# aclyde11/molecular-VAE

Measured on AMD Instinct MI355X. Metric: molecules/s (ELBO fwd+bwd+step), higher is better.
Workload: dtype bf16

## Files before the change

### molecular-vae_amd/csrc/capi.hip

```cpp
#include "common.hpp"
#include "kernels.hpp"

int rnn_fwd_impl(const mvae_rnn_fwd_desc* d, hipStream_t st);
int rnn_bwd_impl(const mvae_rnn_bwd_desc* d, hipStream_t st);
size_t rnn_bwd_workspace_bytes(const mvae_rnn_bwd_desc* d);

thread_local const void* mvae_tls_status = nullptr;

extern "C" {

int mvae_abi_version(void) { return MVAE_ABI_VERSION; }
size_t mvae_struct_size(int which) {
  switch (which) {
    case 0: return sizeof(mvae_rnn_fwd_desc);
    case 1: return sizeof(mvae_rnn_bwd_desc);
    case 2: return sizeof(mvae_gemm_tn_problem);
    case 3: return sizeof(mvae_pack_job);
    case 4: return sizeof(mvae_gemm_tn_f32_problem);
    default: return 0;
  }
}

int mvae_knob_int(const char* name, int dflt) {
  const char* v = name ? mvae_knob(name) : nullptr;
  return v ? atoi(v) : dflt;
}

const char* mvae_status_string(int status) {
  switch (status) {
    case MVAE_OK: return "ok";
    case MVAE_ERR_INVALID: return "invalid argument";
    case MVAE_ERR_WORKSPACE: return "workspace too small";
    case MVAE_ERR_UNSUPPORTED: return "unsupported combination";
    default: return status > 0 ? hipGetErrorString((hipError_t)status) : "unknown status";
  }
}

size_t mvae_gemm_nt_workspace(int M, int N, int K, int dtype_ab) { return gemm_nt_workspace_bytes(M, N, K, dtype_ab); }

int mvae_gemm_nt(int dtype_ab, int M, int N, int K, const void* A, int64_t lda, const void* B, int64_t ldb, void* C, int64_t ldc,
                 int dtype_c, const float* bias, int act, int accumulate, void* ws, size_t ws_bytes, void* stream) {
  return launch_gemm_nt(dtype_ab, M, N, K, A, lda, B, ldb, C, ldc, dtype_c, bias, act, accumulate, ws, ws_bytes, (hipStream_t)stream);
}

size_t mvae_gemm_tn_workspace(int M, int N, int K, int dtype_ab) {
  return dtype_ab == MVAE_BF16 ? gemm_tn_workspace_bytes(M, N, K) : dtype_ab == MVAE_F32 ? gemm_tn_f32_workspace_bytes(M, N, K) : 0;
}

int mvae_gemm_tn(int dtype_ab, int M, int N, int K, const void* A, int64_t lda, const void* B, int64_t ldb, void* C, int64_t ldc,
                 int dtype_c, const float* bias, int act, int accumulate, void* ws, size_t ws_bytes, void* stream) {
  if (dtype_ab == MVAE_F32) {
    if (dtype_c != MVAE_F32 || bias || act != MVAE_ACT_NONE) return MVAE_ERR_UNSUPPORTED;
    return launch_gemm_tn_f32(M, N, K, (const float*)A, lda, 0, 0, (const float*)B, ldb, 0, 0, (float*)C, ldc, accumulate, ws, ws_bytes, (hipStream_t)stream);
  }
  if (dtype_ab != MVAE_BF16) return MVAE_ERR_UNSUPPORTED;
  return launch_gemm_tn_bf16(M, N, K, A, lda, B, ldb, C, ldc, dtype_c, bias, act, accumulate, ws, ws_bytes, (hipStream_t)stream);
}

int mvae_gemm_tn_f32_colsum(int M, int N, int K, const float* A, int64_t lda, const float* B, int64_t ldb, float* C, int64_t ldc, int accumulate,
                            float* colsum_out, int colsum_accumulate, void* ws, size_t ws_bytes, void* stream) {
  if (!colsum_out) return MVAE_ERR_INVALID;
  return launch_gemm_tn_f32(M, N, K, A, lda, 0, 0, B, ldb, 0, 0, C, ldc, accumulate, ws, ws_bytes, (hipStream_t)stream, false, colsum_out, colsum_accumulate);
}

size_t mvae_gemm_tn_colsum_workspace(int M, int N, int K) { return gemm_tn_colsum_supported(M, N, K) ? gemm_tn_colsum_workspace_bytes(M, N, K) : 0; }
int mvae_gemm_tn_colsum_supported(int M, int N, int K) { return gemm_tn_colsum_supported(M, N, K) ? 1 : 0; }
int mvae_gemm_tn_colsum(int M, int N, int K, const void* A, int64_t lda, const void* B, int64_t ldb, float* C, int64_t ldc, int accumulate,
                        float* colsum_out, int colsum_accumulate, void* ws, size_t ws_bytes, void* stream) {
  if (!colsum_out) return MVAE_ERR_INVALID;
  return launch_gemm_tn_bf16_colsum(M, N, K, A, lda, B, ldb, C, ldc, MVAE_F32, nullptr, MVAE_ACT_NONE, accumulate, colsum_out, colsum_accumulate,
                                    ws, ws_bytes, (hipStream_t)stream);
}

int mvae_dropout_keep(uint32_t seed, uint32_t idx, float p) {
  uint32_t h = idx * 0x9E3779B1u ^ seed;
  h ^= h >> 16; h *= 0x85EBCA6Bu; h ^= h >> 13; h *= 0xC2B2AE35u; h ^= h >> 16;
  return h >= (uint32_t)((double)p * 4294967296.0) ? 1 : 0;
}

int mvae_rnn_fwd(const mvae_rnn_fwd_desc* d, void* stream, const void** status_out) {
  mvae_tls_status = nullptr;
  const int rc = (d && d->persist_ws && !d->no_spin && rnn_persist_fwd_supported(d))
                     ? rnn_persist_fwd(d, d->persist_ws, d->persist_ws_bytes, (hipStream_t)stream)
                     : rnn_fwd_impl(d, (hipStream_t)stream);
  if (status_out) *status_out = rc == MVAE_OK ? mvae_tls_status : nullptr;
  return rc;
}
size_t mvae_rnn_fwd_persist_workspace(const mvae_rnn_fwd_desc* d) {
  if (!d) return 0;
  if (rnn_persist_fwd_supported(d)) return rnn_persist_fwd_workspace_bytes(d->T);
  return rnn_rowres_fwd_pipe_workspace(d);
}
int mvae_rnn_bwd(const mvae_rnn_bwd_desc* d, void* stream, const void** status_out) {
  mvae_tls_status = nullptr;
  const int rc = (d && d->persist_ws && !d->no_spin && rnn_persist_bwd_supported(d))
                     ? rnn_persist_bwd(d, d->persist_ws, d->persist_ws_bytes, (hipStream_t)stream)
                     : rnn_bwd_impl(d, (hipStream_t)stream);
  if (status_out) *status_out = rc == MVAE_OK ? mvae_tls_status : nullptr;
  return rc;
}
size_t mvae_rnn_bwd_persist_workspace(const mvae_rnn_bwd_desc* d) { return (d && rnn_persist_bwd_supported(d)) ? rnn_persist_bwd_workspace_bytes(d->T) : 0; }
size_t mvae_rnn_bwd_workspace(const mvae_rnn_bwd_desc* d) { return rnn_bwd_workspace_bytes(d); }

}
```

### molecular-vae_amd/csrc/kernels.hpp

```cpp
#pragma once
#include <atomic>
#include <hip/hip_runtime.h>
#include <stddef.h>
#include "../../include/mvae.h"

size_t gemm_nt_workspace_bytes(int M, int N, int K, int dtype);
int launch_gemm_nt(int dtype, int M, int N, int K, const void* A, long lda, const void* B, long ldb, void* C, long ldc,
                   int c_dtype, const float* bias, int act, int accumulate, void* ws, size_t ws_bytes, hipStream_t st);
int launch_gemm_nt_grouped(int dtype, int M, int N, int K, const void* A, long lda, int a_group, long a_gstride, long a_total,
                           const void* B, long ldb, void* C, long ldc, int c_dtype, const float* bias, int act, int accumulate,
                           void* ws, size_t ws_bytes, hipStream_t st);
size_t gemm_tn_f32_workspace_bytes(int M, int N, int R);
int launch_gemm_tn_f32(int M, int N, int R, const float* A, long lda, int a_group, long a_gstride, const float* B, long ldb, int b_group,
                       long b_gstride, float* C, long ldc, int accumulate, void* ws, size_t ws_bytes, hipStream_t st, bool x3 = false,
                       float* colsum_out = nullptr, int colsum_acc = 0);
size_t gemm_tn_workspace_bytes(int M, int N, int K);
int launch_gemm_tn_bf16(int M, int N, int K, const void* A, long lda, const void* B, long ldb, void* C, long ldc, int c_dtype,
                        const float* bias, int act, int accumulate, void* ws, size_t ws_bytes, hipStream_t st);
bool gemm_tn_colsum_supported(int M, int N, int K);
size_t gemm_tn_colsum_workspace_bytes(int M, int N, int K);
int launch_gemm_tn_bf16_colsum(int M, int N, int K, const void* A, long lda, const void* B, long ldb, void* C, long ldc, int c_dtype,
                               const float* bias, int act, int accumulate, float* colsum_out, int colsum_acc, void* ws, size_t ws_bytes,
                               hipStream_t st);
int launch_cast_transpose(int dsrc, int ddst, int R, int C, const void* src, long lds_, void* dst, long ldd, void* dstT,
                          long ldt, hipStream_t st);
size_t colsum_workspace_bytes(int M, int N);
int launch_colsum(int M, int N, const float* X, long ldx, float* out, void* ws, size_t ws_bytes, hipStream_t st);
int launch_selu_bwd(long n, float* dy, const float* y, hipStream_t st);

extern thread_local const void* mvae_tls_status;
constexpr int MVAE_MAX_DEVICES = 64;

bool rnn_persist_fwd_supported(const mvae_rnn_fwd_desc* d);
size_t rnn_persist_fwd_workspace_bytes(int T);
int rnn_persist_fwd(const mvae_rnn_fwd_desc* d, void* ws, size_t ws_bytes, hipStream_t st);
bool rnn_persist_bwd_supported(const mvae_rnn_bwd_desc* d);
size_t rnn_persist_bwd_workspace_bytes(int T);
int rnn_persist_bwd(const mvae_rnn_bwd_desc* d, void* ws, size_t ws_bytes, hipStream_t st);
size_t rnn_rowres_fwd_pipe_workspace(const mvae_rnn_fwd_desc* d);
```

### molecular-vae_amd/csrc/rnn.hip

```cpp
#include "tile_pipe.hpp"
#include "kernels.hpp"
#include <stdlib.h>

template <typename T> __device__ __forceinline__ void load8(const T* p, float (&v)[8]);
template <> __device__ __forceinline__ void load8<float>(const float* p, float (&v)[8]) {
  const float4 a = *reinterpret_cast<const float4*>(p), b = *reinterpret_cast<const float4*>(p + 4);
  v[0] = a.x; v[1] = a.y; v[2] = a.z; v[3] = a.w; v[4] = b.x; v[5] = b.y; v[6] = b.z; v[7] = b.w;
}
template <> __device__ __forceinline__ void load8<bf16_t>(const bf16_t* p, float (&v)[8]) {
  const uint4 u = *reinterpret_cast<const uint4*>(p);
  const uint32_t w[4] = {u.x, u.y, u.z, u.w};
#pragma unroll
  for (int i = 0; i < 4; ++i) { v[2 * i] = __builtin_bit_cast(float, w[i] << 16); v[2 * i + 1] = __builtin_bit_cast(float, w[i] & 0xffff0000u); }
}
template <typename T> __device__ __forceinline__ void store8(T* p, const float (&v)[8]);
template <> __device__ __forceinline__ void store8<float>(float* p, const float (&v)[8]) {
  *reinterpret_cast<float4*>(p) = make_float4(v[0], v[1], v[2], v[3]);
  *reinterpret_cast<float4*>(p + 4) = make_float4(v[4], v[5], v[6], v[7]);
}
template <> __device__ __forceinline__ void store8<bf16_t>(bf16_t* p, const float (&v)[8]) {
  uint4 u;
  u.x = (uint32_t)f2bf(v[0]) | ((uint32_t)f2bf(v[1]) << 16); u.y = (uint32_t)f2bf(v[2]) | ((uint32_t)f2bf(v[3]) << 16);
  u.z = (uint32_t)f2bf(v[4]) | ((uint32_t)f2bf(v[5]) << 16); u.w = (uint32_t)f2bf(v[6]) | ((uint32_t)f2bf(v[7]) << 16);
  *reinterpret_cast<uint4*>(p) = u;
}
template <typename T> __device__ __forceinline__ void ldn(const T* p, float (&v)[8], int n, bool vec) {
  if (vec && n == 8) { load8<T>(p, v); return; }
#pragma unroll
  for (int e = 0; e < 8; ++e) v[e] = (e < n) ? TT<T>::ld(p + e) : 0.f;
}
template <typename T> __device__ __forceinline__ void stn(T* p, const float (&v)[8], int n, bool vec) {
  if (vec && n == 8) { store8<T>(p, v); return; }
#pragma unroll
  for (int e = 0; e < 8; ++e) if (e < n) TT<T>::st(p + e, v[e]);
}

template <typename T> __device__ __forceinline__ float act_sigmoid(float x);
template <typename T> __device__ __forceinline__ float act_tanh(float x);
template <> __device__ __forceinline__ float act_sigmoid<float>(float x) { return 1.f / (1.f + expf(-x)); }
template <> __device__ __forceinline__ float act_tanh<float>(float x) { return tanhf(x); }
template <> __device__ __forceinline__ float act_sigmoid<bf16_t>(float x) { return __builtin_amdgcn_rcpf(1.f + __expf(-x)); }
template <> __device__ __forceinline__ float act_tanh<bf16_t>(float x) { return fmaf(-2.f, __builtin_amdgcn_rcpf(1.f + __expf(2.f * x)), 1.f); }

__device__ __forceinline__ int xcd_remap_r(int bid, int n) {
  const int q = n >> 3, r = n & 7, x = bid & 7, i = bid >> 3;
  return (x < r ? x * (q + 1) : r * (q + 1) + (x - r) * q) + i;
}

struct DropArgs { float scale; uint32_t thresh, seed; };
__host__ __device__ __forceinline__ uint32_t drop_hash(uint32_t seed, uint32_t idx) {
  uint32_t h = idx * 0x9E3779B1u ^ seed;
  h ^= h >> 16; h *= 0x85EBCA6Bu; h ^= h >> 13; h *= 0xC2B2AE35u; h ^= h >> 16;
  return h;
}
__device__ __forceinline__ float drop_factor(const DropArgs& da, const uint8_t* mask, uint32_t idx0, long off) {
  const bool keep = mask ? (mask[off] != 0) : (drop_hash(da.seed, idx0 + (uint32_t)off) >= da.thresh);
  return keep ? da.scale : 0.f;
}

struct StepTaskF {
  const void *A0, *A1, *W0, *W1;
  long lda0, lda1, ldw0, ldw1;
  int K0, K1;
  const float* add; long add_ld;
  const float* add_tbl;
  const int64_t* add_idx; long add_idx_ld; int add_rows;
  const float* bias;
  const float* c_prev; float* c_out;
  void* c_save;
  void* h_out; long ldh;
  void* g_out;
  const void* hprev_t0;
  int t;
  void* h_drop;
  const uint8_t* dmask;
  uint32_t didx0;
};
struct StepArgsF { StepTaskF t[MVAE_MAX_LAYERS]; const int* lengths; int ntask, B, H, tiles_m, tiles_j, dbg, vec, cell, gru3; DropArgs drop; };

template <typename T, int BM, int BJ, int NBUF, bool WS = false>
__global__ __launch_bounds__(WS ? 512 : 256) void lstm_step_fwd_kernel(StepArgsF p) {
  constexpr bool PIPE = NBUF > 0;
  constexpr int NTHR = WS ? 512 : 256;
  static_assert(!WS || NBUF > 0, "wave specialisation needs the LDS-direct ring");
  extern __shared__ __attribute__((aligned(16))) char smem[];
  static_assert(BJ == 32 || BJ == 64, "hidden units per tile");
  constexpr int JS = BJ / 32;
  constexpr int BN = 4 * BJ, WM = BM / 2, MI = WM / 16, NI = 4 * JS;
  const int tid = threadIdx.x, lane = tid & 63, wave = (tid >> 6) & 3, wm = wave >> 1, wj = wave & 1;
  const int per_task = p.tiles_m * p.tiles_j;
  const int bid = xcd_remap_r(blockIdx.x, p.ntask * per_task);
  const int task = bid / per_task;
  const int rem = bid - task * per_task;
  const int tj = rem / p.tiles_m, tm = rem - tj * p.tiles_m;
  const StepTaskF& q = p.t[task];
  const int m0 = tm * BM, j0 = tj * BJ, H = p.H, B = p.B;

  f32x4 acc[MI][NI];
#pragma unroll
  for (int i = 0; i < MI; ++i)
#pragma unroll
    for (int g = 0; g < NI; ++g) acc[i][g] = f32x4{0.f, 0.f, 0.f, 0.f};

#ifdef MVAE_TUNING
  const bool run_main = !(p.dbg & 2);
#else
  constexpr bool run_main = true;
#endif
  if (run_main) {
  if constexpr (PIPE) {
    PipeSeg<BM, BN> s0, s1;
    const uint32_t sz = (uint32_t)sizeof(T);
    const int skip0 = p.gru3 ? 3 : -1, skip1 = p.gru3 ? 2 : -1;
    {
      const uint32_t lda = (uint32_t)q.lda0 * sz, ldw = (uint32_t)q.ldw0 * sz;
      auto offA = [&](int r) -> uint32_t { const int gm = m0 + r; return gm < B ? (uint32_t)gm * lda : PIPE_OOB; };
      auto offB = [&](int r) -> uint32_t { const int g = r / BJ, j = j0 + (r - g * BJ); return (j < H && g != skip0) ? (uint32_t)(g * H + j) * ldw : PIPE_OOB; };
      pipe_seg_init<T, BM, BN>(s0, q.A0, (uint32_t)B * lda, q.W0, (uint32_t)(4 * H) * ldw, offA, offB, q.K0, tid & 255);
    }
    {
      const uint32_t lda = (uint32_t)q.lda1 * sz, ldw = (uint32_t)q.ldw1 * sz;
      auto offA = [&](int r) -> uint32_t { const int gm = m0 + r; return gm < B ? (uint32_t)gm * lda : PIPE_OOB; };
      auto offB = [&](int r) -> uint32_t { const int g = r / BJ, j = j0 + (r - g * BJ); return (j < H && g != skip1) ? (uint32_t)(g * H + j) * ldw : PIPE_OOB; };
      pipe_seg_init<T, BM, BN>(s1, q.A1, (uint32_t)B * lda, q.W1, (uint32_t)(4 * H) * ldw, offA, offB, q.K1, tid & 255);
    }
    if constexpr (WS) tile_gemm_ws<T, BM, BN, MI, NI, (NBUF > 0 ? NBUF : 3), JS, BJ>(smem, s0, s1, wm * WM, wj * (BJ / 2), acc, tid);
    else tile_gemm_pipe<T, BM, BN, MI, NI, (NBUF > 0 ? NBUF : 3), JS, BJ>(smem, s0, s1, wm * WM, wj * (BJ / 2), acc, tid);
  } else {
    int brow[NI];
#pragma unroll
    for (int g = 0; g < NI; ++g) brow[g] = (g / JS) * BJ + wj * (BJ / 2) + (g % JS) * 16;
    if (q.A0 != nullptr) {
      const T* A = reinterpret_cast<const T*>(q.A0);
      const T* W = reinterpret_cast<const T*>(q.W0);
      const long lda = q.lda0, ldw = q.ldw0;
      auto rowA = [&](int r) -> const T* { const int gm = m0 + r; return gm < B ? A + (long)gm * lda : nullptr; };
      auto rowB = [&](int r) -> const T* { const int g = r / BJ, j = j0 + (r - g * BJ); return (j < H && !(p.gru3 && g == 3)) ? W + ((long)g * H + j) * ldw : nullptr; };
      tile_gemm_segment<T, BM, BN, MI, NI>(smem, rowA, rowB, 0, q.K0, wm * WM, brow, acc, tid);
    }
    if (q.A1 != nullptr) {
      const T* A = reinterpret_cast<const T*>(q.A1);
      const T* W = reinterpret_cast<const T*>(q.W1);
      const long lda = q.lda1, ldw = q.ldw1;
      auto rowA = [&](int r) -> const T* { const int gm = m0 + r; return gm < B ? A + (long)gm * lda : nullptr; };
      auto rowB = [&](int r) -> const T* { const int g = r / BJ, j = j0 + (r - g * BJ); return (j < H && !(p.gru3 && g == 2)) ? W + ((long)g * H + j) * ldw : nullptr; };
      tile_gemm_segment<T, BM, BN, MI, NI>(smem, rowA, rowB, 0, q.K1, wm * WM, brow, acc, tid);
    }
  }
  }
#ifdef MVAE_TUNING
  if (p.dbg & 1) { if (acc[0][0][0] == 12345.678f) q.c_out[0] = 1.f; return; }
#endif

  constexpr int SJ = BJ + 4;
  constexpr int GPRW = BJ / 8;
  constexpr int NIT = (BM * GPRW + NTHR - 1) / NTHR;
  float* stg = reinterpret_cast<float*>(smem);
  const int g8 = tid % GPRW;
  const int j8 = j0 + g8 * 8;
  const int n = (H - j8 < 8) ? (H - j8) : 8;
  const bool vec = p.vec != 0;
  const bool fast = vec && n == 8 && m0 + BM <= B && (BM * GPRW) % NTHR == 0;
  float bias[4][8], cpv[NIT][8];
  if (fast) {
    const float* bsrc = q.bias ? q.bias : q.c_out;
#pragma unroll
    for (int g = 0; g < 4; ++g) load8<float>(bsrc + g * H + j8, bias[g]);
    if (q.c_prev) {
#pragma unroll
      for (int it = 0; it < NIT; ++it) load8<float>(q.c_prev + (long)(m0 + tid / GPRW + it * (NTHR / GPRW)) * H + j8, cpv[it]);
    } else if (q.hprev_t0) {
#pragma unroll
      for (int it = 0; it < NIT; ++it)
        load8<T>(reinterpret_cast<const T*>(q.hprev_t0) + (long)(m0 + tid / GPRW + it * (NTHR / GPRW)) * q.lda1 + j8, cpv[it]);
    } else {
#pragma unroll
      for (int it = 0; it < NIT; ++it)
#pragma unroll
        for (int e = 0; e < 8; ++e) cpv[it][e] = 0.f;
    }
    if (!q.bias) {
#pragma unroll
      for (int g = 0; g < 4; ++g)
#pragma unroll
        for (int e = 0; e < 8; ++e) bias[g][e] = 0.f;
    }
  } else {
#pragma unroll
  for (int g = 0; g < 4; ++g) {
    if (q.bias && n > 0) ldn<float>(q.bias + g * H + j8, bias[g], n, vec);
    else {
#pragma unroll
      for (int e = 0; e < 8; ++e) bias[g][e] = 0.f;
    }
  }
#pragma unroll
  for (int it = 0; it < NIT; ++it) {
    const int lrow = tid / GPRW + it * (NTHR / GPRW);
    const int row = m0 + lrow;
    const bool live = n > 0 && lrow < BM && row < B;
    if (live && q.c_prev) ldn<float>(q.c_prev + (long)row * H + j8, cpv[it], n, vec);
    else if (live && q.hprev_t0) ldn<T>(reinterpret_cast<const T*>(q.hprev_t0) + (long)row * q.lda1 + j8, cpv[it], n, vec);
    else {
#pragma unroll
      for (int e = 0; e < 8; ++e) cpv[it][e] = 0.f;
    }
  }
  }
  if (!WS || tid < 256) {
    const int lr = lane & 15, lq = lane >> 4;
#pragma unroll
    for (int i = 0; i < MI; ++i)
#pragma unroll
      for (int ni = 0; ni < NI; ++ni)
#pragma unroll
        for (int r = 0; r < 4; ++r) {
          const int row = wm * WM + i * 16 + lq * 4 + r;
          stg[(row * 4 + ni / JS) * SJ + wj * (BJ / 2) + (ni % JS) * 16 + lr] = acc[i][ni][r];
        }
  }
  __syncthreads();
  if (n <= 0) return;
  T* hout = reinterpret_cast<T*>(q.h_out);
  T* gout = reinterpret_cast<T*>(q.g_out);
  T* csave = reinterpret_cast<T*>(q.c_save);
  auto rows = [&](auto fast_tag, auto add_tag) {
  constexpr bool FAST = decltype(fast_tag)::value, HAS_ADD = decltype(add_tag)::value;
  auto ld32 = [&](const float* src, float (&v)[8]) { if constexpr (FAST) load8<float>(src, v); else ldn<float>(src, v, n, vec); };
  auto st32 = [&](float* dst, const float (&v)[8]) { if constexpr (FAST) store8<float>(dst, v); else stn<float>(dst, v, n, vec); };
  auto stT = [&](T* dst, const float (&v)[8]) { if constexpr (FAST) store8<T>(dst, v); else stn<T>(dst, v, n, vec); };
#pragma unroll
  for (int it = 0; it < NIT; ++it) {
    const int lrow = tid / GPRW + it * (NTHR / GPRW);
    const int row = m0 + lrow;
    if constexpr (!FAST) { if (lrow >= BM || row >= B) continue; }
    float pre[4][8];
#pragma unroll
    for (int g = 0; g < 4; ++g) {
      const float* s = stg + (lrow * 4 + g) * SJ + g8 * 8;
      const float4 a = *reinterpret_cast<const float4*>(s), b = *reinterpret_cast<const float4*>(s + 4);
      pre[g][0] = a.x + bias[g][0]; pre[g][1] = a.y + bias[g][1]; pre[g][2] = a.z + bias[g][2]; pre[g][3] = a.w + bias[g][3];
      pre[g][4] = b.x + bias[g][4]; pre[g][5] = b.y + bias[g][5]; pre[g][6] = b.z + bias[g][6]; pre[g][7] = b.w + bias[g][7];
    }
    if constexpr (HAS_ADD) {
    if (q.add_tbl) {
      long id = q.add_idx[(long)row * q.add_idx_ld];
      id = id < 0 ? 0 : (id >= q.add_rows ? q.add_rows - 1 : id);
      const float* tr = q.add_tbl + id * 4L * H + j8;
#pragma unroll
      for (int g = 0; g < 4; ++g) {
        float a[8], b[8];
        ld32(tr + g * H, a);
        if (q.add) {
          ld32(q.add + (long)row * q.add_ld + g * H + j8, b);
#pragma unroll
          for (int e = 0; e < 8; ++e) a[e] += b[e];
        }
#pragma unroll
        for (int e = 0; e < 8; ++e) pre[g][e] += a[e];
      }
    } else if (q.add) {
#pragma unroll
      for (int g = 0; g < 4; ++g) {
        float a[8];
        ld32(q.add + (long)row * q.add_ld + g * H + j8, a);
#pragma unroll
        for (int e = 0; e < 8; ++e) pre[g][e] += a[e];
      }
    }
    }
    const float (&cp)[8] = cpv[it];
    T* g4 = gout + (long)row * 4 * H + j8;
    if (p.cell == MVAE_CELL_LSTM) {
      float gi[8], gf[8], gg[8], go[8], c[8], h[8];
#pragma unroll
      for (int e = 0; e < 8; ++e) {
        gi[e] = act_sigmoid<T>(pre[0][e]); gf[e] = act_sigmoid<T>(pre[1][e]); gg[e] = act_tanh<T>(pre[2][e]); go[e] = act_sigmoid<T>(pre[3][e]);
        c[e] = gf[e] * cp[e] + gi[e] * gg[e];
        h[e] = go[e] * act_tanh<T>(c[e]);
      }
      st32(q.c_out + (long)row * H + j8, c);
      stT(hout + (long)row * q.ldh + j8, h);
      if (q.h_drop) {
        float hd[8];
#pragma unroll
        for (int e = 0; e < 8; ++e) hd[e] = (e < n) ? h[e] * drop_factor(p.drop, q.dmask, q.didx0, (long)row * H + j8 + e) : 0.f;
        stT(reinterpret_cast<T*>(q.h_drop) + (long)row * q.ldh + j8, hd);
      }
      if (gout) {
        stT(csave + (long)row * H + j8, c);
        stT(g4, gi); stT(g4 + H, gf); stT(g4 + 2 * H, gg); stT(g4 + 3 * H, go);
      }
    } else {
      const bool valid = p.lengths ? (q.t < p.lengths[row]) : true;
      float gr[8], gz[8], gn[8], hs_[8], hseq[8];
#pragma unroll
      for (int e = 0; e < 8; ++e) {
        gr[e] = act_sigmoid<T>(pre[0][e]); gz[e] = act_sigmoid<T>(pre[1][e]);
        gn[e] = act_tanh<T>(pre[2][e] + gr[e] * pre[3][e]);
        const float hn = (1.f - gz[e]) * gn[e] + gz[e] * cp[e];
        hs_[e] = valid ? hn : cp[e];
        hseq[e] = valid ? hn : 0.f;
      }
      st32(q.c_out + (long)row * H + j8, hs_);
      stT(hout + (long)row * q.ldh + j8, hseq);
      if (q.h_drop) {
        float hd[8];
#pragma unroll
        for (int e = 0; e < 8; ++e) hd[e] = (e < n) ? hseq[e] * drop_factor(p.drop, q.dmask, q.didx0, (long)row * H + j8 + e) : 0.f;
        stT(reinterpret_cast<T*>(q.h_drop) + (long)row * q.ldh + j8, hd);
      }
      if (gout) { stT(g4, gr); stT(g4 + H, gz); stT(g4 + 2 * H, gn); stT(g4 + 3 * H, pre[3]); }
    }
  }
  };
  const bool has_add = q.add != nullptr || q.add_tbl != nullptr;
  if (fast) { if (has_add) rows(std::true_type{}, std::true_type{}); else rows(std::true_type{}, std::false_type{}); }
  else { if (has_add) rows(std::false_type{}, std::true_type{}); else rows(std::false_type{}, std::false_type{}); }
}

template <int BMW, int BNB, int NBUF, bool WS = false>
__global__ __launch_bounds__(WS ? 512 : BMW * 2) void lstm_step_fwd_gm_kernel(StepArgsF p) {
  using T = bf16_t;
  extern __shared__ __attribute__((aligned(16))) char smem[];
  static_assert(BMW == 256 || BMW == 128, "weight rows per tile: 64 or 32 units x 4 gates");
  static_assert(!WS || BMW == 128, "loader / consumer split: the 4-wave tile only");
  constexpr int NT = BMW * 2;
  constexpr int BU = BMW / 4;
  constexpr int MI = 8, NI = BNB / 64;
  const int tid = threadIdx.x, lane = tid & 63, wave = WS ? ((tid >> 6) & 3) : (tid >> 6), wm = wave >> 2, wn = wave & 3;
  const int per_task = p.tiles_m * p.tiles_j;
  const int bid = xcd_remap_r(blockIdx.x, p.ntask * per_task);
  const int task = bid / per_task;
  const int rem = bid - task * per_task;
  const int tj = rem / p.tiles_m, tm = rem - tj * p.tiles_m;
  const StepTaskF& q = p.t[task];
  const int n0 = tm * BNB, j0 = tj * BU, H = p.H, B = p.B;

  const int lq = lane >> 4, lc = lane & 15;
  const int ub = j0 + 32 * wm + 8 * lq;
  constexpr bool BIAS_FIRST = (BMW == 256 && BNB == 256);
  auto load_bias = [&](float (&bias)[4][8]) {
    if (q.bias) {
#pragma unroll
      for (int g = 0; g < 4; ++g) load8<float>(q.bias + g * H + ub, bias[g]);
    } else {
#pragma unroll
      for (int g = 0; g < 4; ++g)
#pragma unroll
        for (int e = 0; e < 8; ++e) bias[g][e] = 0.f;
    }
  };
  f32x4 acc[MI][NI];
  if constexpr (BIAS_FIRST) {
    float bias[4][8];
    load_bias(bias);
#pragma unroll
    for (int ni = 0; ni < NI; ++ni)
#pragma unroll
      for (int g = 0; g < 4; ++g)
#pragma unroll
        for (int e = 0; e < 8; ++e) acc[2 * g + (e >> 2)][ni][e & 3] = bias[g][e];
  } else {
#pragma unroll
    for (int i = 0; i < MI; ++i)
#pragma unroll
      for (int g = 0; g < NI; ++g) acc[i][g] = f32x4{0.f, 0.f, 0.f, 0.f};
  }

  float cpa[NI][8];
  auto load_cprev_all = [&]() {
    const float* cpsrc = q.c_prev ? q.c_prev : q.c_out;
#pragma unroll
    for (int ni = 0; ni < NI; ++ni) {
      const int row = n0 + wn * (16 * NI) + ni * 16 + lc;
      load8<float>(cpsrc + (long)(row < B ? row : B - 1) * H + ub, cpa[ni]);
    }
  };
  if constexpr (BIAS_FIRST) load_cprev_all();

#ifdef MVAE_TUNING
  const bool run_main = !(p.dbg & 2);
#else
  constexpr bool run_main = true;
#endif
  if (run_main) {
    PipeSeg<BMW, BNB, NT> s0, s1;
    auto wrow = [&](int r) -> int {
      const int mi = (r >> 4) & 7, j = r & 15;
      return (mi >> 1) * H + j0 + 32 * (r >> 7) + 8 * (j >> 2) + 4 * (mi & 1) + (j & 3);
    };
    {
      const uint32_t lda = (uint32_t)q.lda0 * 2u, ldw = (uint32_t)q.ldw0 * 2u;
      auto offW = [&](int r) -> uint32_t { return (uint32_t)wrow(r) * ldw; };
      auto offX = [&](int r) -> uint32_t { const int gn = n0 + r; return gn < B ? (uint32_t)gn * lda : PIPE_OOB; };
      pipe_seg_init<T, BMW, BNB, NT>(s0, q.W0, (uint32_t)(4 * H) * ldw, q.A0, (uint32_t)B * lda, offW, offX, q.K0, WS ? (tid & 255) : tid);
      if (q.A0 == nullptr) s0.nk = 0;
    }
    {
      const uint32_t lda = (uint32_t)q.lda1 * 2u, ldw = (uint32_t)q.ldw1 * 2u;
      auto offW = [&](int r) -> uint32_t { return (uint32_t)wrow(r) * ldw; };
      auto offX = [&](int r) -> uint32_t { const int gn = n0 + r; return gn < B ? (uint32_t)gn * lda : PIPE_OOB; };
      pipe_seg_init<T, BMW, BNB, NT>(s1, q.W1, (uint32_t)(4 * H) * ldw, q.A1, (uint32_t)B * lda, offW, offX, q.K1, WS ? (tid & 255) : tid);
      if (q.A1 == nullptr) s1.nk = 0;
    }
    if constexpr (WS) tile_gemm_ws<T, BMW, BNB, MI, NI, NBUF, NI, 0>(smem, s0, s1, 0, wn * (16 * NI), acc, tid);
    else tile_gemm_pipe_all<T, BMW, BNB, MI, NI, NBUF, NT>(smem, s0, s1, wm * 128, wn * (16 * NI), acc, tid);
  }
  if constexpr (WS) { if (tid >= 256) return; }
#ifdef MVAE_TUNING
  if (p.dbg & 1) { if (acc[0][0][0] == 12345.678f) q.c_out[0] = 1.f; return; }
#endif

  if constexpr (!BIAS_FIRST) {
    float bias[4][8];
    load_bias(bias);
#pragma unroll
    for (int ni = 0; ni < NI; ++ni)
#pragma unroll
      for (int g = 0; g < 4; ++g)
#pragma unroll
        for (int e = 0; e < 8; ++e) acc[2 * g + (e >> 2)][ni][e & 3] += bias[g][e];
  }
  T* hout = reinterpret_cast<T*>(q.h_out);
  T* gout = reinterpret_cast<T*>(q.g_out);
  T* csave = reinterpret_cast<T*>(q.c_save);
  if constexpr (!BIAS_FIRST) load_cprev_all();
  const bool has_cprev = q.c_prev != nullptr;
  auto epilogue = [&](auto has_add, auto full_tile) {
#pragma unroll
  for (int ni = 0; ni < NI; ++ni) {
    const int row = n0 + wn * (16 * NI) + ni * 16 + lc;
    if constexpr (!decltype(full_tile)::value) { if (row >= B) continue; }
    float cp[8];
#pragma unroll
    for (int e = 0; e < 8; ++e) cp[e] = has_cprev ? cpa[ni][e] : 0.f;
    float pre[4][8];
#pragma unroll
    for (int g = 0; g < 4; ++g)
#pragma unroll
      for (int e = 0; e < 8; ++e) pre[g][e] = acc[2 * g + (e >> 2)][ni][e & 3];
    if constexpr (decltype(has_add)::value) {
#pragma unroll
      for (int g = 0; g < 4; ++g) {
        float a[8];
        load8<float>(q.add + (long)row * q.add_ld + g * H + ub, a);
#pragma unroll
        for (int e = 0; e < 8; ++e) pre[g][e] += a[e];
      }
    }
    float gi[8], gf[8], gg[8], go[8], c[8], h[8];
#pragma unroll
    for (int e = 0; e < 8; ++e) {
      gi[e] = act_sigmoid<T>(pre[0][e]); gf[e] = act_sigmoid<T>(pre[1][e]); gg[e] = act_tanh<T>(pre[2][e]); go[e] = act_sigmoid<T>(pre[3][e]);
      c[e] = gf[e] * cp[e] + gi[e] * gg[e];
      h[e] = go[e] * act_tanh<T>(c[e]);
    }
#ifdef MVAE_TUNING
    const int srow = (p.dbg & 4) ? n0 + (row & 15) : row;
    const bool sgate = !(p.dbg & 8);
#else
    const int srow = row;
    constexpr bool sgate = true;
#endif
    store8<float>(q.c_out + (long)srow * H + ub, c);
    store8<T>(hout + (long)srow * q.ldh + ub, h);
    if (gout) {
      T* g4 = gout + (long)srow * 4 * H + ub;
      store8<T>(csave + (long)srow * H + ub, c);
      if (sgate) { store8<T>(g4, gi); store8<T>(g4 + H, gf); store8<T>(g4 + 2 * H, gg); store8<T>(g4 + 3 * H, go); }
    }
  }
  };
  const bool full = n0 + BNB <= B;
  if (q.add) { if (full) epilogue(std::true_type{}, std::true_type{}); else epilogue(std::true_type{}, std::false_type{}); }
  else { if (full) epilogue(std::false_type{}, std::true_type{}); else epilogue(std::false_type{}, std::false_type{}); }
}

struct StepTaskB {
  const void *A0, *A1, *W0, *W1;
  long lda0, lda1, ldw0, ldw1;
  int K0, K1;
  const float* dy; long dy_ld;
  const void* gates; const void* c; const void* c_prev;
  const float* dc_in; float* dc_out;
  void* dG; long ldg;
  const void* h_prev; long ldhp;
  float* dh0;
  int t;
  int seg1_full;
  int drop;
  const uint8_t* dmask;
  uint32_t didx0;
};
struct StepArgsB { StepTaskB t[MVAE_MAX_LAYERS]; const int* lengths; float* partial; int ntask, B, H, tiles_m, tiles_n, dbg, vec, cell, split, gru3; DropArgs drop; };

template <typename T>
__device__ __forceinline__ void bwd_cell_group(const StepArgsB& p, const StepTaskB& q, int row, int j8, int n, bool vec, float (&dh)[8]) {
  const int H = p.H;
  const T* gates = reinterpret_cast<const T*>(q.gates);
  const T* cs = reinterpret_cast<const T*>(q.c);
  const T* csp = reinterpret_cast<const T*>(q.c_prev);
  T* dG = reinterpret_cast<T*>(q.dG);
  const long o = (long)row * H + j8;
  float dci[8];
  if (q.dc_in) ldn<float>(q.dc_in + o, dci, n, vec);
  else {
#pragma unroll
    for (int e = 0; e < 8; ++e) dci[e] = 0.f;
  }
  if (p.cell == MVAE_CELL_LSTM) {
    if (q.dy) {
      float a[8];
      ldn<float>(q.dy + (long)row * q.dy_ld + j8, a, n, vec);
#pragma unroll
      for (int e = 0; e < 8; ++e) dh[e] += a[e];
    }
    float gi[8], gf[8], gg[8], go[8], c[8], cp[8];
    const T* g4 = gates + (long)row * 4 * H + j8;
    ldn<T>(g4, gi, n, vec); ldn<T>(g4 + H, gf, n, vec); ldn<T>(g4 + 2 * H, gg, n, vec); ldn<T>(g4 + 3 * H, go, n, vec);
    ldn<T>(cs + o, c, n, vec);
    if (csp) ldn<T>(csp + o, cp, n, vec);
    else {
#pragma unroll
      for (int e = 0; e < 8; ++e) cp[e] = 0.f;
    }
    float di[8], df[8], dg[8], dO[8], dco[8];
#pragma unroll
    for (int e = 0; e < 8; ++e) {
      const float tc = act_tanh<T>(c[e]);
      const float d_o = dh[e] * tc;
      const float dc = dh[e] * go[e] * (1.f - tc * tc) + dci[e];
      dco[e] = dc * gf[e];
      di[e] = dc * gg[e] * gi[e] * (1.f - gi[e]);
      df[e] = dc * cp[e] * gf[e] * (1.f - gf[e]);
      dg[e] = dc * gi[e] * (1.f - gg[e] * gg[e]);
      dO[e] = d_o * go[e] * (1.f - go[e]);
    }
    stn<float>(q.dc_out + o, dco, n, vec);
    T* d4 = dG + (long)row * q.ldg + j8;
    stn<T>(d4, di, n, vec); stn<T>(d4 + H, df, n, vec); stn<T>(d4 + 2 * H, dg, n, vec); stn<T>(d4 + 3 * H, dO, n, vec);
  } else {
#pragma unroll
    for (int e = 0; e < 8; ++e) dh[e] += dci[e];
    if (q.gates == nullptr) {
      stn<float>(q.dh0 + o, dh, n, vec);
      return;
    }
    const bool valid = p.lengths ? (q.t < p.lengths[row]) : true;
    float dpr[8], dpz[8], dpn[8], dpnr[8], carry[8];
    if (valid) {
      if (q.dy) {
        float a[8];
        ldn<float>(q.dy + (long)row * q.dy_ld + j8, a, n, vec);
#pragma unroll
        for (int e = 0; e < 8; ++e) dh[e] += a[e];
      }
      float gr[8], gz[8], gn[8], nh[8], hp[8];
      const T* g4 = gates + (long)row * 4 * H + j8;
      ldn<T>(g4, gr, n, vec); ldn<T>(g4 + H, gz, n, vec); ldn<T>(g4 + 2 * H, gn, n, vec); ldn<T>(g4 + 3 * H, nh, n, vec);
      if (q.h_prev) ldn<T>(reinterpret_cast<const T*>(q.h_prev) + (long)row * q.ldhp + j8, hp, n, vec);
      else {
#pragma unroll
        for (int e = 0; e < 8; ++e) hp[e] = 0.f;
      }
#pragma unroll
      for (int e = 0; e < 8; ++e) {
        const float dn = dh[e] * (1.f - gz[e]);
        const float dz = dh[e] * (hp[e] - gn[e]);
        dpn[e] = dn * (1.f - gn[e] * gn[e]);
        dpr[e] = dpn[e] * nh[e] * gr[e] * (1.f - gr[e]);
        dpz[e] = dz * gz[e] * (1.f - gz[e]);
        dpnr[e] = dpn[e] * gr[e];
        carry[e] = dh[e] * gz[e];
      }
    } else {
#pragma unroll
      for (int e = 0; e < 8; ++e) { dpr[e] = 0.f; dpz[e] = 0.f; dpn[e] = 0.f; dpnr[e] = 0.f; carry[e] = dh[e]; }
    }
    stn<float>(q.dc_out + o, carry, n, vec);
    T* d4 = dG + (long)row * q.ldg + j8;
    stn<T>(d4, dpr, n, vec); stn<T>(d4 + H, dpz, n, vec); stn<T>(d4 + 2 * H, dpn, n, vec); stn<T>(d4 + 3 * H, dpnr, n, vec);
  }
}

struct BwdOps { float dci[8], dy[8], g[4][8], c[8], cp[8]; };

template <typename T, bool FAST>
__device__ __forceinline__ void bwd_cell_load(const StepArgsB& p, const StepTaskB& q, int row, int j8, int n, bool vec, BwdOps& r) {
  const int H = p.H;
  const T* gates = reinterpret_cast<const T*>(q.gates);
  const long o = (long)row * H + j8;
  if constexpr (FAST) {
    load8<float>((q.dc_in ? q.dc_in : q.dc_out) + o, r.dci);
    if (gates == nullptr) return;
    load8<float>(q.dy ? q.dy + (long)row * q.dy_ld + j8 : q.dc_out + o, r.dy);
    const T* g4 = gates + (long)row * 4 * H + j8;
    load8<T>(g4, r.g[0]); load8<T>(g4 + H, r.g[1]); load8<T>(g4 + 2 * H, r.g[2]); load8<T>(g4 + 3 * H, r.g[3]);
    if (p.cell == MVAE_CELL_LSTM) {
      const T* cs = reinterpret_cast<const T*>(q.c);
      const T* csp = reinterpret_cast<const T*>(q.c_prev);
      load8<T>(cs + o, r.c);
      load8<T>((csp ? csp : cs) + o, r.cp);
    } else {
      load8<T>(q.h_prev ? reinterpret_cast<const T*>(q.h_prev) + (long)row * q.ldhp + j8 : g4, r.cp);
    }
  } else {
    if (q.dc_in) ldn<float>(q.dc_in + o, r.dci, n, vec);
    if (gates == nullptr) return;
    if (q.dy) ldn<float>(q.dy + (long)row * q.dy_ld + j8, r.dy, n, vec);
    const T* g4 = gates + (long)row * 4 * H + j8;
    ldn<T>(g4, r.g[0], n, vec); ldn<T>(g4 + H, r.g[1], n, vec); ldn<T>(g4 + 2 * H, r.g[2], n, vec); ldn<T>(g4 + 3 * H, r.g[3], n, vec);
    if (p.cell == MVAE_CELL_LSTM) {
      ldn<T>(reinterpret_cast<const T*>(q.c) + o, r.c, n, vec);
      if (q.c_prev) ldn<T>(reinterpret_cast<const T*>(q.c_prev) + o, r.cp, n, vec);
    } else if (q.h_prev) ldn<T>(reinterpret_cast<const T*>(q.h_prev) + (long)row * q.ldhp + j8, r.cp, n, vec);
  }
}

template <typename T, bool FAST>
__device__ __forceinline__ void bwd_cell_finish(const StepArgsB& p, const StepTaskB& q, int row, int j8, int n, bool vec, const BwdOps& r,
                                                float (&dh)[8]) {
  const int H = p.H;
  T* dG = reinterpret_cast<T*>(q.dG);
  const long o = (long)row * H + j8;
  auto st32 = [&](float* dst, const float (&v)[8]) { if constexpr (FAST) store8<float>(dst, v); else stn<float>(dst, v, n, vec); };
  auto stT = [&](T* dst, const float (&v)[8]) { if constexpr (FAST) store8<T>(dst, v); else stn<T>(dst, v, n, vec); };
  const bool has_dci = q.dc_in != nullptr, has_dy = q.dy != nullptr;
  float dci[8];
#pragma unroll
  for (int e = 0; e < 8; ++e) dci[e] = has_dci ? r.dci[e] : 0.f;
  if (p.cell == MVAE_CELL_LSTM) {
#pragma unroll
    for (int e = 0; e < 8; ++e) dh[e] += has_dy ? r.dy[e] : 0.f;
    const bool has_cp = q.c_prev != nullptr;
    float di[8], df[8], dg[8], dO[8], dco[8];
#pragma unroll
    for (int e = 0; e < 8; ++e) {
      const float gi = r.g[0][e], gf = r.g[1][e], gg = r.g[2][e], go = r.g[3][e], cp = has_cp ? r.cp[e] : 0.f;
      const float tc = act_tanh<T>(r.c[e]);
      const float d_o = dh[e] * tc;
      const float dc = dh[e] * go * (1.f - tc * tc) + dci[e];
      dco[e] = dc * gf;
      di[e] = dc * gg * gi * (1.f - gi);
      df[e] = dc * cp * gf * (1.f - gf);
      dg[e] = dc * gi * (1.f - gg * gg);
      dO[e] = d_o * go * (1.f - go);
    }
    st32(q.dc_out + o, dco);
    T* d4 = dG + (long)row * q.ldg + j8;
    stT(d4, di); stT(d4 + H, df); stT(d4 + 2 * H, dg); stT(d4 + 3 * H, dO);
  } else {
#pragma unroll
    for (int e = 0; e < 8; ++e) dh[e] += dci[e];
    if (q.gates == nullptr) {
      st32(q.dh0 + o, dh);
      return;
    }
    const bool valid = p.lengths ? (q.t < p.lengths[row]) : true;
    const bool has_hp = q.h_prev != nullptr;
    float dpr[8], dpz[8], dpn[8], dpnr[8], carry[8];
    if (valid) {
#pragma unroll
      for (int e = 0; e < 8; ++e) dh[e] += has_dy ? r.dy[e] : 0.f;
#pragma unroll
      for (int e = 0; e < 8; ++e) {
        const float gr = r.g[0][e], gz = r.g[1][e], gn = r.g[2][e], nh = r.g[3][e], hp = has_hp ? r.cp[e] : 0.f;
        const float dn = dh[e] * (1.f - gz);
        const float dz = dh[e] * (hp - gn);
        dpn[e] = dn * (1.f - gn * gn);
        dpr[e] = dpn[e] * nh * gr * (1.f - gr);
        dpz[e] = dz * gz * (1.f - gz);
        dpnr[e] = dpn[e] * gr;
        carry[e] = dh[e] * gz;
      }
    } else {
#pragma unroll
      for (int e = 0; e < 8; ++e) { dpr[e] = 0.f; dpz[e] = 0.f; dpn[e] = 0.f; dpnr[e] = 0.f; carry[e] = dh[e]; }
    }
    st32(q.dc_out + o, carry);
    T* d4 = dG + (long)row * q.ldg + j8;
    stT(d4, dpr); stT(d4 + H, dpz); stT(d4 + 2 * H, dpn); stT(d4 + 3 * H, dpnr);
  }
}

struct BwdRaw { float4 dci[2], dy[2]; uint4 g[4], c, cp; };
template <bool HAS_DY>
__device__ __forceinline__ void bwd_raw_load(const StepArgsB& p, const StepTaskB& q, int row, int j8, BwdRaw& r) {
  const int H = p.H;
  const bf16_t* gates = reinterpret_cast<const bf16_t*>(q.gates);
  const long o = (long)row * H + j8;
  const float* dsrc = (q.dc_in ? q.dc_in : q.dc_out) + o;
  r.dci[0] = *reinterpret_cast<const float4*>(dsrc); r.dci[1] = *reinterpret_cast<const float4*>(dsrc + 4);
  if (gates == nullptr) return;
  if constexpr (HAS_DY) {
    const float* ysrc = q.dy ? q.dy + (long)row * q.dy_ld + j8 : q.dc_out + o;
    r.dy[0] = *reinterpret_cast<const float4*>(ysrc); r.dy[1] = *reinterpret_cast<const float4*>(ysrc + 4);
  }
  const bf16_t* g4 = gates + (long)row * 4 * H + j8;
  r.g[0] = *reinterpret_cast<const uint4*>(g4); r.g[1] = *reinterpret_cast<const uint4*>(g4 + H);
  r.g[2] = *reinterpret_cast<const uint4*>(g4 + 2 * H); r.g[3] = *reinterpret_cast<const uint4*>(g4 + 3 * H);
  if (p.cell == MVAE_CELL_LSTM) {
    const bf16_t* cs = reinterpret_cast<const bf16_t*>(q.c);
    const bf16_t* csp = reinterpret_cast<const bf16_t*>(q.c_prev);
    r.c = *reinterpret_cast<const uint4*>(cs + o);
    r.cp = *reinterpret_cast<const uint4*>((csp ? csp : cs) + o);
  } else {
    r.cp = *reinterpret_cast<const uint4*>(q.h_prev ? reinterpret_cast<const bf16_t*>(q.h_prev) + (long)row * q.ldhp + j8 : g4);
  }
}
__device__ __forceinline__ void unpack8(const uint4& u, float (&v)[8]) {
  const uint32_t w[4] = {u.x, u.y, u.z, u.w};
#pragma unroll
  for (int i = 0; i < 4; ++i) { v[2 * i] = __builtin_bit_cast(float, w[i] << 16); v[2 * i + 1] = __builtin_bit_cast(float, w[i] & 0xffff0000u); }
}
template <bool HAS_DY>
__device__ __forceinline__ void bwd_raw_unpack(const BwdRaw& r, BwdOps& o) {
  o.dci[0] = r.dci[0].x; o.dci[1] = r.dci[0].y; o.dci[2] = r.dci[0].z; o.dci[3] = r.dci[0].w;
  o.dci[4] = r.dci[1].x; o.dci[5] = r.dci[1].y; o.dci[6] = r.dci[1].z; o.dci[7] = r.dci[1].w;
  if constexpr (HAS_DY) {
    o.dy[0] = r.dy[0].x; o.dy[1] = r.dy[0].y; o.dy[2] = r.dy[0].z; o.dy[3] = r.dy[0].w;
    o.dy[4] = r.dy[1].x; o.dy[5] = r.dy[1].y; o.dy[6] = r.dy[1].z; o.dy[7] = r.dy[1].w;
  } else {
#pragma unroll
    for (int e = 0; e < 8; ++e) o.dy[e] = 0.f;
  }
#pragma unroll
  for (int g = 0; g < 4; ++g) unpack8(r.g[g], o.g[g]);
  unpack8(r.c, o.c); unpack8(r.cp, o.cp);
}

template <typename T, int BM, int BN, int NBUF, bool WS = false, bool DROP = false, int SPLITMODE = -1, int PREF = 0>
__global__ __launch_bounds__(WS ? 512 : 256) void lstm_step_bwd_kernel(StepArgsB p) {
  constexpr bool PIPE = NBUF > 0;
  constexpr int NTHR = WS ? 512 : 256;
  static_assert(!WS || NBUF > 0, "wave specialisation needs the LDS-direct ring");
  extern __shared__ __attribute__((aligned(16))) char smem[];
  constexpr int WM = BM / 2, WN = BN / 2, MI = WM / 16, NI = WN / 16;
  const int tid = threadIdx.x, lane = tid & 63, wave = (tid >> 6) & 3, wm = wave >> 1, wn = wave & 1;
  const int per_task = p.tiles_m * p.tiles_n;
  const int nsp = p.split ? p.split : 1;
  const int bid = xcd_remap_r(blockIdx.x, p.ntask * per_task * nsp);
  const int task2 = bid / per_task;
  const int task = task2 / nsp;
  const int sp = task2 - task * nsp;
  const int seg = (nsp == 4) ? (sp >> 1) : sp;
  const int half = (nsp == 4) ? (sp & 1) : 0;
  const int rem = bid - task2 * per_task;
  int tn = rem / p.tiles_m, tm = rem - tn * p.tiles_m;
  if (p.tiles_m >= 16 && (p.tiles_m & 7) == 0 && (p.tiles_n & 3) == 0) {
    const int blk = rem >> 5, in = rem & 31, mb = p.tiles_m >> 3;
    const int tnb = blk / mb, tmb = blk - tnb * mb;
    tn = 4 * tnb + (in >> 3); tm = 8 * tmb + (in & 7);
  }
  const StepTaskB& q = p.t[task];
  const int m0 = tm * BM, n0 = tn * BN, H = p.H, B = p.B;
  if (p.split && (seg == 0 ? q.A0 == nullptr : q.A1 == nullptr)) return;

  f32x4 acc[MI][NI];
#pragma unroll
  for (int i = 0; i < MI; ++i)
#pragma unroll
    for (int n = 0; n < NI; ++n) acc[i][n] = f32x4{0.f, 0.f, 0.f, 0.f};

  if constexpr (PREF != 0) {
    static_assert(WS && NBUF > 0 && SPLITMODE == 0 && !DROP && sizeof(T) == 2, "prefetching form: fused, wave-specialised, bf16");
    constexpr bool HAS_DY = PREF == 1;
    constexpr int SN = BN + 4, GPR = BN / 8, RPI = NTHR / GPR, NIT = BM / RPI;
    static_assert(BM % RPI == 0, "whole row groups per thread");
    PipeSeg<BM, BN> s0, s1;
#ifdef MVAE_TUNING
    const int am0 = (p.dbg & 4) ? 0 : m0, an0 = (p.dbg & 4) ? 0 : n0;
#else
    const int am0 = m0, an0 = n0;
#endif
    {
      const uint32_t lda = (uint32_t)q.lda0 * 2u, ldw = (uint32_t)q.ldw0 * 2u;
      auto offA = [&](int r) -> uint32_t { return (uint32_t)(am0 + r) * lda; };
      auto offB = [&](int r) -> uint32_t { return (uint32_t)(an0 + r) * ldw; };
      pipe_seg_init<T, BM, BN>(s0, q.A0, (uint32_t)B * lda, q.W0, (uint32_t)H * ldw, offA, offB, p.gru3 ? 3 * H : q.K0, tid & 255);
      if (p.gru3) { s0.hole_st = (int)(2 * H * 2 / KB); s0.hole_bytes = (uint32_t)H * 2u; }
    }
    {
      const uint32_t lda = (uint32_t)q.lda1 * 2u, ldw = (uint32_t)q.ldw1 * 2u;
      auto offA = [&](int r) -> uint32_t { return (uint32_t)(am0 + r) * lda; };
      auto offB = [&](int r) -> uint32_t { return (uint32_t)(an0 + r) * ldw; };
      pipe_seg_init<T, BM, BN>(s1, q.A1, (uint32_t)B * lda, q.W1, (uint32_t)H * ldw, offA, offB, (p.gru3 && !q.seg1_full) ? 3 * H : q.K1, tid & 255);
    }
    const int nk = s0.nk + s1.nk;
    const int wv = __builtin_amdgcn_readfirstlane(tid >> 6);
    const int g8 = tid % GPR, j8 = n0 + g8 * 8, row0 = m0 + tid / GPR;
    float* stg = reinterpret_cast<float*>(smem);
    BwdRaw raw[NIT];
    auto finish_all = [&]() {
#pragma unroll
      for (int it = 0; it < NIT; ++it) {
        const int lrow = tid / GPR + it * RPI;
        const float* sp_ = stg + lrow * SN + g8 * 8;
        const float4 a = *reinterpret_cast<const float4*>(sp_), b = *reinterpret_cast<const float4*>(sp_ + 4);
        float dh[8] = {a.x, a.y, a.z, a.w, b.x, b.y, b.z, b.w};
        BwdOps o;
        bwd_raw_unpack<HAS_DY>(raw[it], o);
        bwd_cell_finish<T, true>(p, q, m0 + lrow, j8, 8, true, o, dh);
      }
    };
#ifdef MVAE_TUNING
    const bool run_main = !(p.dbg & 2);
#else
    constexpr bool run_main = true;
#endif
    if (wv >= 4) {
      constexpr int NTAIL = NIT * (HAS_DY ? 10 : 8);
      const bool tail_form = p.cell == MVAE_CELL_LSTM && nk >= NBUF && run_main;
      if (tail_form) {
        tile_gemm_ws_loader_tail<T, BM, BN, NBUF, NTAIL>(smem, s0, s1, wv - 4, [&]() {
#pragma unroll
          for (int it = 0; it < NIT; ++it) bwd_raw_load<HAS_DY>(p, q, row0 + it * RPI, j8, raw[it]);
        });
        ws_barrier();
      } else {
#ifdef MVAE_TUNING
      if (!(p.dbg & 64))
#endif
#pragma unroll
      for (int it = 0; it < NIT; ++it) bwd_raw_load<HAS_DY>(p, q, row0 + it * RPI, j8, raw[it]);
      if (nk > 0 && run_main) { tile_gemm_ws_loader<T, BM, BN, NBUF>(smem, s0, s1, wv - 4, p.dbg); ws_barrier(); }
      }
#ifdef MVAE_TUNING
      if (p.dbg & 1) return;
#endif
      __syncthreads();
      finish_all();
    } else {
#ifdef MVAE_TUNING
      if (!(p.dbg & 64))
#endif
      bwd_raw_load<HAS_DY>(p, q, row0, j8, raw[0]);
      if (nk > 0 && run_main) { tile_gemm_ws_consumer<T, BM, BN, MI, NI, NBUF, NI, 0, true>(smem, nk, wm * WM, wn * WN, acc, lane, p.dbg); ws_barrier(); }
#ifdef MVAE_TUNING
      if (p.dbg & 1) { if (acc[0][0][0] == 12345.678f) q.dc_out[0] = 1.f; return; }
#endif
      const int lr = lane & 15, lq = lane >> 4;
#pragma unroll
      for (int i = 0; i < MI; ++i)
#pragma unroll
        for (int n = 0; n < NI; ++n)
#pragma unroll
          for (int r = 0; r < 4; ++r) stg[(wm * WM + i * 16 + lq * 4 + r) * SN + wn * WN + n * 16 + lr] = acc[i][n][r];
#pragma unroll
      for (int it = 1; it < NIT; ++it) bwd_raw_load<HAS_DY>(p, q, row0 + it * RPI, j8, raw[it]);
      __syncthreads();
      finish_all();
    }
    return;
  }
  const bool fused_drop = DROP && q.drop && !p.split && q.A1 != nullptr;
  auto scale_drop = [&]() {
#pragma unroll
    for (int i = 0; i < MI; ++i)
#pragma unroll
      for (int n = 0; n < NI; ++n)
#pragma unroll
        for (int r = 0; r < 4; ++r) {
          const int row = m0 + wm * WM + i * 16 + (lane >> 4) * 4 + r, col = n0 + wn * WN + n * 16 + (lane & 15);
          if (row < B && col < H) acc[i][n][r] *= drop_factor(p.drop, q.dmask, q.didx0, (long)row * H + col);
        }
  };
#ifdef MVAE_TUNING
  const bool run_main = !(p.dbg & 2);
#else
  constexpr bool run_main = true;
#endif
  if (run_main) {
  if constexpr (PIPE) {
    PipeSeg<BM, BN> s0, s1;
    const uint32_t sz = (uint32_t)sizeof(T);
    {
      const uint32_t lda = (uint32_t)q.lda0 * sz, ldw = (uint32_t)q.ldw0 * sz;
      auto offA = [&](int r) -> uint32_t { const int gm = m0 + r; return gm < B ? (uint32_t)gm * lda : PIPE_OOB; };
      auto offB = [&](int r) -> uint32_t { const int gn = n0 + r; return gn < H ? (uint32_t)gn * ldw : PIPE_OOB; };
      int kh = (nsp == 4) ? q.K0 / 2 : q.K0, ko = half * kh * (int)sz;
      if (p.gru3) {
        if (nsp == 4) { kh = half ? H : 2 * H; ko = half ? 3 * H * (int)sz : 0; }
        else kh = 3 * H;
      }
      pipe_seg_init<T, BM, BN>(s0, q.A0 ? reinterpret_cast<const char*>(q.A0) + ko : nullptr, (uint32_t)B * lda - ko,
                               reinterpret_cast<const char*>(q.W0) + ko, (uint32_t)H * ldw - ko, offA, offB, kh, tid & 255);
      if (p.gru3 && nsp != 4) { s0.hole_st = (int)(2 * H * sz / KB); s0.hole_bytes = (uint32_t)H * sz; }
      if (p.split && seg == 1) s0.nk = 0;
    }
    {
      const uint32_t lda = (uint32_t)q.lda1 * sz, ldw = (uint32_t)q.ldw1 * sz;
      auto offA = [&](int r) -> uint32_t { const int gm = m0 + r; return gm < B ? (uint32_t)gm * lda : PIPE_OOB; };
      auto offB = [&](int r) -> uint32_t { const int gn = n0 + r; return gn < H ? (uint32_t)gn * ldw : PIPE_OOB; };
      const int k1 = (p.gru3 && !q.seg1_full) ? 3 * H : q.K1;
      const int kh = (nsp == 4) ? k1 / 2 : k1, ko = half * kh * (int)sz;
      pipe_seg_init<T, BM, BN>(s1, q.A1 ? reinterpret_cast<const char*>(q.A1) + ko : nullptr, (uint32_t)B * lda - ko,
                               reinterpret_cast<const char*>(q.W1) + ko, (uint32_t)H * ldw - ko, offA, offB, kh, tid & 255);
      if (p.split && seg == 0) s1.nk = 0;
    }
    if constexpr (DROP) {
      const int nk0 = s0.nk;
      s0.nk = 0;
      tile_gemm_pipe<T, BM, BN, MI, NI, (NBUF > 0 ? NBUF : 3), NI, 0>(smem, s0, s1, wm * WM, wn * WN, acc, tid);
      if (fused_drop) scale_drop();
      s0.nk = nk0; s1.nk = 0;
      tile_gemm_pipe<T, BM, BN, MI, NI, (NBUF > 0 ? NBUF : 3), NI, 0>(smem, s0, s1, wm * WM, wn * WN, acc, tid);
    } else {
      if constexpr (WS) tile_gemm_ws<T, BM, BN, MI, NI, (NBUF > 0 ? NBUF : 3), NI, 0, (BM * BN <= 128 * 128)>(smem, s0, s1, wm * WM, wn * WN, acc, tid);
      else tile_gemm_pipe<T, BM, BN, MI, NI, (NBUF > 0 ? NBUF : 3), NI, 0>(smem, s0, s1, wm * WM, wn * WN, acc, tid);
    }
  } else {
    int brow[NI];
#pragma unroll
    for (int n = 0; n < NI; ++n) brow[n] = wn * WN + n * 16;
    if (fused_drop && q.A1 != nullptr) {
      const T* A = reinterpret_cast<const T*>(q.A1);
      const T* W = reinterpret_cast<const T*>(q.W1);
      const long lda = q.lda1, ldw = q.ldw1;
      auto rowA = [&](int r) -> const T* { const int gm = m0 + r; return gm < B ? A + (long)gm * lda : nullptr; };
      auto rowB = [&](int r) -> const T* { const int gn = n0 + r; return gn < H ? W + (long)gn * ldw : nullptr; };
      tile_gemm_segment<T, BM, BN, MI, NI>(smem, rowA, rowB, 0, p.gru3 ? 3 * H : q.K1, wm * WM, brow, acc, tid);
      scale_drop();
    }
    if (q.A0 != nullptr) {
      const T* A = reinterpret_cast<const T*>(q.A0);
      const T* W = reinterpret_cast<const T*>(q.W0);
      const long lda = q.lda0, ldw = q.ldw0;
      auto rowA = [&](int r) -> const T* { const int gm = m0 + r; return gm < B ? A + (long)gm * lda : nullptr; };
      auto rowB = [&](int r) -> const T* { const int gn = n0 + r; return gn < H ? W + (long)gn * ldw : nullptr; };
      if (p.gru3) {
        tile_gemm_segment<T, BM, BN, MI, NI>(smem, rowA, rowB, 0, 2 * H, wm * WM, brow, acc, tid);
        tile_gemm_segment<T, BM, BN, MI, NI>(smem, rowA, rowB, 3 * H, 4 * H, wm * WM, brow, acc, tid);
      } else tile_gemm_segment<T, BM, BN, MI, NI>(smem, rowA, rowB, 0, q.K0, wm * WM, brow, acc, tid);
    }
    if (!fused_drop && q.A1 != nullptr) {
      const T* A = reinterpret_cast<const T*>(q.A1);
      const T* W = reinterpret_cast<const T*>(q.W1);
      const long lda = q.lda1, ldw = q.ldw1;
      auto rowA = [&](int r) -> const T* { const int gm = m0 + r; return gm < B ? A + (long)gm * lda : nullptr; };
      auto rowB = [&](int r) -> const T* { const int gn = n0 + r; return gn < H ? W + (long)gn * ldw : nullptr; };
      tile_gemm_segment<T, BM, BN, MI, NI>(smem, rowA, rowB, 0, p.gru3 ? 3 * H : q.K1, wm * WM, brow, acc, tid);
    }
  }
  }
#ifdef MVAE_TUNING
  if (p.dbg & 1) { if (acc[0][0][0] == 12345.678f) q.dc_out[0] = 1.f; return; }
#endif

  constexpr int SN = BN + 4;
  float* stg = reinterpret_cast<float*>(smem);
  if (!WS || tid < 256) {
    const int lr = lane & 15, lq = lane >> 4;
#pragma unroll
    for (int i = 0; i < MI; ++i)
#pragma unroll
      for (int n = 0; n < NI; ++n)
#pragma unroll
        for (int r = 0; r < 4; ++r) stg[(wm * WM + i * 16 + lq * 4 + r) * SN + wn * WN + n * 16 + lr] = acc[i][n][r];
  }
  __syncthreads();
  constexpr int GPR = BN / 8;
  const int g8 = tid % GPR;
  const int j8 = n0 + g8 * 8;
  if (j8 >= H) return;
  const int n = (H - j8 < 8) ? (H - j8) : 8;
  const bool vec = p.vec != 0;
  if ((SPLITMODE == 1) || (SPLITMODE == -1 && p.split)) {
    float* part = p.partial + ((long)(task * nsp + sp) * B) * H;
#pragma unroll
    for (int it = 0; it < (BM * GPR + NTHR - 1) / NTHR; ++it) {
      const int lrow = tid / GPR + it * (NTHR / GPR);
      const int row = m0 + lrow;
      if (lrow >= BM || row >= B) continue;
      const float* sp = stg + lrow * SN + g8 * 8;
      float* dst = part + (long)row * H + j8;
      *reinterpret_cast<float4*>(dst) = *reinterpret_cast<const float4*>(sp);
      *reinterpret_cast<float4*>(dst + 4) = *reinterpret_cast<const float4*>(sp + 4);
    }
    return;
  }
  if constexpr (SPLITMODE != 1) {
  constexpr int NIT = (BM * GPR + NTHR - 1) / NTHR;
  auto read_dh = [&](int lrow, float (&dh)[8]) {
    const float* s = stg + lrow * SN + g8 * 8;
    const float4 a = *reinterpret_cast<const float4*>(s), b = *reinterpret_cast<const float4*>(s + 4);
    dh[0] = a.x; dh[1] = a.y; dh[2] = a.z; dh[3] = a.w; dh[4] = b.x; dh[5] = b.y; dh[6] = b.z; dh[7] = b.w;
  };
  if (vec && n == 8 && m0 + BM <= B && (BM * GPR) % NTHR == 0) {
    BwdOps ops[2];
    bwd_cell_load<T, true>(p, q, m0 + tid / GPR, j8, 8, true, ops[0]);
#pragma unroll
    for (int it = 0; it < NIT; ++it) {
      const int lrow = tid / GPR + it * (NTHR / GPR);
      if (it + 1 < NIT) bwd_cell_load<T, true>(p, q, m0 + lrow + NTHR / GPR, j8, 8, true, ops[(it + 1) & 1]);
      float dh[8];
      read_dh(lrow, dh);
      bwd_cell_finish<T, true>(p, q, m0 + lrow, j8, 8, true, ops[it & 1], dh);
    }
    return;
  }
#pragma unroll
  for (int it = 0; it < NIT; ++it) {
    const int lrow = tid / GPR + it * (NTHR / GPR);
    const int row = m0 + lrow;
    if (lrow >= BM || row >= B) continue;
    float dh[8];
    read_dh(lrow, dh);
    bwd_cell_group<T>(p, q, row, j8, n, vec, dh);
  }
  }
}

template <typename T>
__global__ __launch_bounds__(256) void lstm_bwd_epi_kernel(StepArgsB p) {
  const int H = p.H, B = p.B;
  const int gpr = H / 8;
  const long per_task = (long)B * gpr;
  const long gid = (long)blockIdx.x * 256 + threadIdx.x;
  if (gid >= per_task * p.ntask) return;
  const int task = (int)(gid / per_task);
  const long rem = gid - (long)task * per_task;
  const int row = (int)(rem / gpr), j8 = (int)(rem - (long)row * gpr) * 8;
  const StepTaskB& q = p.t[task];
  float dh[8] = {0.f, 0.f, 0.f, 0.f, 0.f, 0.f, 0.f, 0.f};
  const int nsp = p.split, per_seg = nsp >> 1;
  const float* p0 = p.partial + ((long)(task * nsp) * B + row) * H + j8;
  for (int s = 0; s < nsp; ++s) {
    if ((s / per_seg == 0) ? (q.A0 == nullptr) : (q.A1 == nullptr)) continue;
    float a[8]; load8<float>(p0 + (long)s * B * H, a);
    if (q.drop && s / per_seg == 1) {
#pragma unroll
      for (int e = 0; e < 8; ++e) a[e] *= drop_factor(p.drop, q.dmask, q.didx0, (long)row * H + j8 + e);
    }
#pragma unroll
    for (int e = 0; e < 8; ++e) dh[e] += a[e];
  }
  bwd_cell_group<T>(p, q, row, j8, 8, true, dh);
}

#define MVAE_STEP_LAUNCH(KERN)                                                                                     \
  do {                                                                                                               \
    auto kern = KERN;                                                                                                \
    static bool attr_set = false;                                                                                    \
    if (!attr_set) { MVAE_CHECK_HIP(hipFuncSetAttribute(reinterpret_cast<const void*>(kern), hipFuncAttributeMaxDynamicSharedMemorySize, 160 * 1024)); attr_set = true; } \
    hipLaunchKernelGGL(kern, grid, block, lds, st, a);                                                               \
  } while (0)

static int tune_int(const char* name, int dflt) {
  const char* v = mvae_knob(name);
  return v ? atoi(v) : dflt;
}

static inline const char* adv(const void* p, long elems, int dtype) {
  return reinterpret_cast<const char*>(p) + elems * (dtype == MVAE_BF16 ? 2 : 4);
}
static inline bool al16(const void* p) { return (reinterpret_cast<uintptr_t>(p) & 15) == 0; }

int rnn_rowres_fwd(const mvae_rnn_fwd_desc* d, hipStream_t st);
int rnn_gru_rowres_fwd(const mvae_rnn_fwd_desc* d, hipStream_t st);

int rnn_fwd_impl(const mvae_rnn_fwd_desc* d, hipStream_t st) {
  if (!d) return MVAE_ERR_INVALID;
  if (d->cell != MVAE_CELL_LSTM && d->cell != MVAE_CELL_GRU) return MVAE_ERR_UNSUPPORTED;
  if (d->layers < 1 || d->layers > MVAE_MAX_LAYERS || d->T < 1 || d->B < 1 || d->H < 1) return MVAE_ERR_INVALID;
  if (d->dtype != MVAE_F32 && d->dtype != MVAE_BF16) return MVAE_ERR_INVALID;
  const int NL = d->layers, T = d->T, B = d->B, H = d->H, dt = d->dtype;
  const int epc = (dt == MVAE_BF16) ? 8 : 4;
  const bool gru = d->cell == MVAE_CELL_GRU;
  if (d->lengths && !gru) return MVAE_ERR_UNSUPPORTED;
  const bool infer = !d->gates[0];
  for (int l = 0; l < NL; ++l) {
    if (infer ? (d->gates[l] || d->cs[l]) : ((!gru && !d->cs[l]) || !d->gates[l])) return MVAE_ERR_INVALID;
    if (!d->w_hh[l] || !d->hs[l] || !d->cstate[l]) return MVAE_ERR_INVALID;
    if (l > 0 && !d->w_ih[l]) return MVAE_ERR_INVALID;
    if (d->ldw_hh[l] % epc) return MVAE_ERR_INVALID;
    if (l > 0 && d->ldw_ih[l] % epc) return MVAE_ERR_INVALID;
  }
  if (d->x0 && (!d->w_ih[0] || d->in0 < 1)) return MVAE_ERR_INVALID;
  if (!d->x0 && !d->add0 && !d->add_table) return MVAE_ERR_INVALID;
  if (d->add_table && (!d->add_index || d->add_table_rows < 1 || d->add_index_ld < T)) return MVAE_ERR_INVALID;
  if (d->ldh % epc) return MVAE_ERR_INVALID;
  bool drop = false;
  for (int l = 0; l < NL; ++l) drop = drop || d->hdrop[l] != nullptr;
  if (drop) {
    if (!(d->drop_p > 0.f) || d->drop_p >= 1.f) return MVAE_ERR_INVALID;
    for (int l = 0; l + 1 < NL; ++l) if (!d->hdrop[l]) return MVAE_ERR_INVALID;
  }
  if (!drop) {
    const int rc = rnn_rowres_fwd(d, st);
    if (rc != MVAE_ERR_UNSUPPORTED) return rc;
  }
  if (!drop) {
    const int rc = rnn_gru_rowres_fwd(d, st);
    if (rc != MVAE_ERR_UNSUPPORTED) return rc;
  }
  auto nblk = [&](int bm) { return (long)((B + bm - 1) / bm) * ((H + 31) / 32) * NL; };
  int BM = (nblk(128) >= 256) ? 128 : (nblk(64) >= 256 || dt == MVAE_BF16) ? 64 : 32;
  if (dt == MVAE_BF16) BM = 64;
  BM = tune_int("MVAE_BM", BM);
  if (BM == 32 && dt == MVAE_BF16) BM = 64;
  const int sz = (dt == MVAE_BF16) ? 2 : 4, ke = KB / sz;
  int Hk = H;
  if (d->zero_padded_k && H % ke) {
    const int hp = (H + ke - 1) / ke * ke;
    bool ok = d->ldh >= hp && (!d->h0[0] || d->ldh0 >= hp);
    for (int l = 0; l < NL; ++l) ok = ok && d->ldw_hh[l] >= hp && (l == 0 || d->ldw_ih[l] >= hp);
    if (ok) Hk = hp;
  }
  bool pipe = (Hk % ke == 0) && (d->ldh % (16 / sz) == 0) && ((long)B * d->ldh * sz < (1L << 31)) && (!d->x0 || (d->in0 % ke == 0 && d->x0_ld % (16 / sz) == 0)) &&
              (!d->h0[0] || d->ldh0 % (16 / sz) == 0);
  bool vec = (H % 8 == 0) && (d->ldh % 8 == 0) && (!d->add0 || (al16(d->add0) && d->add0_tstride % 4 == 0)) && (!d->add_table || al16(d->add_table));
  for (int l = 0; l < NL; ++l) {
    if ((4L * H) * d->ldw_hh[l] * sz >= (1L << 31) || d->ldw_hh[l] % (16 / sz)) pipe = false;
    if ((l > 0 || d->x0) && ((4L * H) * d->ldw_ih[l] * sz >= (1L << 31) || d->ldw_ih[l] % (16 / sz))) pipe = false;
    if (!al16(d->hs[l]) || (!gru && !infer && !al16(d->cs[l])) || (!infer && !al16(d->gates[l])) || !al16(d->cstate[l]) || (d->bias[l] && !al16(d->bias[l]))) vec = false;
    if (d->h0[l] && (!al16(d->h0[l]) || d->ldh0 % 8)) vec = false;
  }
  StepArgsF a;
  a.lengths = d->lengths; a.cell = d->cell;
  int BJ = (pipe && dt == MVAE_BF16 && (long)((B + 127) / 128) * ((H + 63) / 64) * NL >= 256) ? 64 : 32;
  BJ = tune_int("MVAE_BJ", BJ);
  if (BJ == 64 && (!pipe || dt != MVAE_BF16)) BJ = 32;
  if (BJ == 64) BM = 128;
  const int gm_knob = tune_int("MVAE_FWD_GM", 1);
  int BMW = 0, BNB = 0;
  for (int l = 0; l < NL && drop; ++l) if (d->hdrop[l] && (!al16(d->hdrop[l]))) vec = false;
  if (gm_knob && !gru && !drop && !d->add_table && dt == MVAE_BF16 && pipe && vec && H % 64 == 0) {
    static const int cand[4][2] = {{256, 256}, {256, 128}, {128, 128}, {128, 64}};
    for (int c = 0; c < 4 && !BMW; ++c) {
      const long tiles = (long)((B + cand[c][1] - 1) / cand[c][1]) * (H / (cand[c][0] / 4)) * NL;
      const bool chosen = gm_knob == 1 && tiles >= 192 && ((c == 0 && B >= 256) || (c == 3 && B >= 64 && B <= 128));
      if (gm_knob == cand[c][0] * 1000 + cand[c][1] || chosen) { BMW = cand[c][0]; BNB = cand[c][1]; }
    }
  }
  if (BMW) { BM = BNB; BJ = BMW / 4; }
  a.B = B; a.H = H; a.tiles_m = (B + BM - 1) / BM; a.tiles_j = (H + BJ - 1) / BJ; a.vec = vec ? 1 : 0;
  a.drop.scale = drop ? 1.f / (1.f - d->drop_p) : 1.f;
  a.drop.thresh = drop ? (uint32_t)((double)d->drop_p * 4294967296.0) : 0u;
  a.drop.seed = d->drop_seed;
  a.gru3 = gru ? 1 : 0;
#ifdef MVAE_TUNING
  a.dbg = tune_int("MVAE_DBG", 0);
#else
  a.dbg = 0;
#endif
  int nbuf_dflt = (BJ == 64) ? 3 : (dt == MVAE_BF16 && BM == 64) ? 3 : 4;
  if (dt == MVAE_BF16 && BM == 64 && BJ == 32 && !BMW) {
    const long nb = (long)((B + BM - 1) / BM) * ((H + BJ - 1) / BJ) * NL, cus = 256;
    if ((nb + 3 * cus - 1) / (3 * cus) < (nb + 2 * cus - 1) / (2 * cus)) nbuf_dflt = 2;
  }
  const int nbuf = pipe ? tune_int("MVAE_NBUF_FWD", nbuf_dflt) : 0;
  size_t lds = (size_t)(nbuf > 0 ? nbuf : 2) * (BM + 4 * BJ) * KB;
  const size_t stage_bytes = (size_t)BM * 4 * (BJ + 4) * sizeof(float);
  if (lds < stage_bytes) lds = stage_bytes;
  for (int dd = 0; dd < T + NL - 1; ++dd) {
    int n = 0;
    for (int l = 0; l < NL; ++l) {
      const int t = dd - l;
      if (t < 0 || t >= T) continue;
      StepTaskF& q = a.t[n++];
      if (l == 0) {
        q.A0 = d->x0 ? adv(d->x0, (long)t * B * d->x0_ld, dt) : nullptr;
        q.lda0 = d->x0_ld; q.K0 = d->in0; q.W0 = d->w_ih[0]; q.ldw0 = d->ldw_ih[0];
        q.add = d->add0 ? d->add0 + (long)t * d->add0_tstride : nullptr;
        q.add_ld = 4L * H;
        q.add_tbl = d->add_table; q.add_idx = d->add_table ? d->add_index + t : nullptr; q.add_idx_ld = d->add_index_ld; q.add_rows = d->add_table_rows;
      } else {
        q.A0 = adv(drop ? d->hdrop[l - 1] : d->hs[l - 1], (long)t * B * d->ldh, dt);
        q.lda0 = d->ldh; q.K0 = Hk; q.W0 = d->w_ih[l]; q.ldw0 = d->ldw_ih[l];
        q.add = nullptr; q.add_ld = 0;
        q.add_tbl = nullptr; q.add_idx = nullptr; q.add_idx_ld = 0; q.add_rows = 0;
      }
      q.A1 = (t > 0) ? adv(d->hs[l], (long)(t - 1) * B * d->ldh, dt) : d->h0[l];
      q.lda1 = (t > 0) ? d->ldh : d->ldh0;
      q.K1 = Hk; q.W1 = d->w_hh[l]; q.ldw1 = d->ldw_hh[l];
      q.bias = d->bias[l];
      q.c_prev = (t > 0) ? d->cstate[l] + (long)((t - 1) & 1) * B * H : nullptr;
      q.c_out = d->cstate[l] + (long)(t & 1) * B * H;
      q.c_save = (gru || infer) ? nullptr : const_cast<char*>(adv(d->cs[l], (long)t * B * H, dt));
      q.hprev_t0 = (gru && t == 0) ? d->h0[l] : nullptr;
      q.t = t;
      q.h_drop = (drop && l + 1 < NL) ? const_cast<char*>(adv(d->hdrop[l], (long)t * B * d->ldh, dt)) : nullptr;
      q.dmask = (drop && d->drop_mask[l]) ? d->drop_mask[l] + ((long)t * B) * H : nullptr;
      q.didx0 = (uint32_t)((((long)l * T + t) * B) * H);
      q.h_out = const_cast<char*>(adv(d->hs[l], (long)t * B * d->ldh, dt)); q.ldh = d->ldh;
      q.g_out = infer ? nullptr : const_cast<char*>(adv(d->gates[l], (long)t * B * 4 * H, dt));
    }
    a.ntask = n;
    dim3 grid(n * a.tiles_m * a.tiles_j), block(256);
    if (BMW) {
      block = dim3(BMW * 2);
      if (BMW == 256 && BNB == 256) {
        lds = 2 * (256 + 256) * KB;
        MVAE_STEP_LAUNCH((lstm_step_fwd_gm_kernel<256, 256, 2>));
      }
      else if (BMW == 256) { lds = 3 * (256 + 128) * KB; MVAE_STEP_LAUNCH((lstm_step_fwd_gm_kernel<256, 128, 3>)); }
      else if (BNB == 128) { lds = 4 * (128 + 128) * KB; MVAE_STEP_LAUNCH((lstm_step_fwd_gm_kernel<128, 128, 4>)); }
      else { lds = 4 * (128 + 64) * KB; block = dim3(512); MVAE_STEP_LAUNCH((lstm_step_fwd_gm_kernel<128, 64, 4, true>)); }
      continue;
    }
#define FWD_CASE(TT_, BM_, NB_) if (BJ == 32 && BM == BM_ && nbuf == NB_) { MVAE_STEP_LAUNCH((lstm_step_fwd_kernel<TT_, BM_, 32, NB_>)); continue; }
    if (BJ == 64 && nbuf == 3) {
      block = dim3(512); MVAE_STEP_LAUNCH((lstm_step_fwd_kernel<bf16_t, 128, 64, 3, true>));
      continue;
    }
    if (dt == MVAE_BF16) {
      FWD_CASE(bf16_t, 128, 0) FWD_CASE(bf16_t, 128, 3) FWD_CASE(bf16_t, 128, 4) FWD_CASE(bf16_t, 128, 5)
      FWD_CASE(bf16_t, 64, 0) FWD_CASE(bf16_t, 64, 2) FWD_CASE(bf16_t, 64, 3) FWD_CASE(bf16_t, 64, 4) FWD_CASE(bf16_t, 64, 5)
    } else {
      FWD_CASE(float, 128, 0) FWD_CASE(float, 128, 4) FWD_CASE(float, 64, 0) FWD_CASE(float, 64, 4) FWD_CASE(float, 32, 0) FWD_CASE(float, 32, 4)
    }
#undef FWD_CASE
    return MVAE_ERR_UNSUPPORTED;
  }
  MVAE_CHECK_HIP(hipGetLastError());
  return MVAE_OK;
}

int rnn_rowres_bwd(const mvae_rnn_bwd_desc* d, hipStream_t st);
int rnn_gru_rowres_bwd(const mvae_rnn_bwd_desc* d, hipStream_t st);
size_t rnn_rowres_bwd_workspace(int layers, int T, int B, int H);

size_t rnn_bwd_workspace_bytes(const mvae_rnn_bwd_desc* d) {
  if (!d || d->layers < 1 || d->B < 1 || d->H < 1 || d->T < 1) return 0;
  const size_t split = (size_t)d->layers * 4 * d->B * d->H * sizeof(float);
  const size_t rowres = rnn_rowres_bwd_workspace(d->layers, d->T, d->B, d->H);
  return split > rowres ? split : rowres;
}

int rnn_bwd_impl(const mvae_rnn_bwd_desc* d, hipStream_t st) {
  if (!d) return MVAE_ERR_INVALID;
  if (d->cell != MVAE_CELL_LSTM && d->cell != MVAE_CELL_GRU) return MVAE_ERR_UNSUPPORTED;
  if (d->layers < 1 || d->layers > MVAE_MAX_LAYERS || d->T < 1 || d->B < 1 || d->H < 1) return MVAE_ERR_INVALID;
  if (d->dtype != MVAE_F32 && d->dtype != MVAE_BF16) return MVAE_ERR_INVALID;
  const int NL = d->layers, T = d->T, B = d->B, H = d->H, dt = d->dtype;
  const int epc = (dt == MVAE_BF16) ? 8 : 4;
  const bool gru = d->cell == MVAE_CELL_GRU;
  if (!d->dy && !d->dy_a && !gru) return MVAE_ERR_INVALID;
  if (d->dy_a && (!d->dy_w || d->dy_k < 128 || d->dy_k % 128 || d->dy_a_ld < d->dy_k || d->dy_w_ld < d->dy_k || d->dy_a_ld % epc || d->dy_w_ld % epc ||
                  ((reinterpret_cast<uintptr_t>(d->dy_a) | reinterpret_cast<uintptr_t>(d->dy_w)) & 15)))
    return MVAE_ERR_INVALID;
  if (d->lengths && !gru) return MVAE_ERR_UNSUPPORTED;
  for (int l = 0; l < NL; ++l) {
    if (!d->w_hhT[l] || (!gru && !d->cs[l]) || !d->gates[l] || !d->dG[l] || !d->dstate[l]) return MVAE_ERR_INVALID;
    if (gru && !d->hs[l]) return MVAE_ERR_INVALID;
    if (l > 0 && !d->w_ihT[l]) return MVAE_ERR_INVALID;
    if (d->ldw_hhT[l] % epc || (l > 0 && d->ldw_ihT[l] % epc)) return MVAE_ERR_INVALID;
  }
  const long ldg = d->ldg;
  if (ldg < 4L * H || ldg % epc) return MVAE_ERR_INVALID;
  const bool drop = d->drop_p > 0.f;
  if (drop && d->drop_p >= 1.f) return MVAE_ERR_INVALID;
  if (!drop) {
    const int rc = rnn_rowres_bwd(d, st);
    if (rc != MVAE_ERR_UNSUPPORTED) return rc;
  }
  if (!drop) {
    const int rc = rnn_gru_rowres_bwd(d, st);
    if (rc != MVAE_ERR_UNSUPPORTED) return rc;
  }
  int BM = 64, BN = 64;
  if (dt == MVAE_F32 && (long)((B + 63) / 64) * ((H + 63) / 64) * NL < 256) { BM = 32; BN = 32; }
  if (!drop) BM = tune_int("MVAE_BM", BM);
  if (BM == 32 && dt == MVAE_BF16) BM = 64;
  if (BM != 32) BN = 64;
  const int sz = (dt == MVAE_BF16) ? 2 : 4, ke = KB / sz;
  bool pipe = ((4 * H) % ke == 0) && ((long)B * ldg * sz < (1L << 31)) && (ldg % (16 / sz) == 0);
  bool vec = (H % 8 == 0) && (ldg % 8 == 0) && (!d->dy || (al16(d->dy) && (d->dy_ld % 4 == 0)));
  for (int l = 0; l < NL; ++l) {
    if ((long)H * d->ldw_hhT[l] * sz >= (1L << 31) || d->ldw_hhT[l] % (16 / sz)) pipe = false;
    if (l > 0 && ((long)H * d->ldw_ihT[l] * sz >= (1L << 31) || d->ldw_ihT[l] % (16 / sz))) pipe = false;
    if ((!gru && !al16(d->cs[l])) || !al16(d->gates[l]) || !al16(d->dG[l]) || !al16(d->dstate[l])) vec = false;
    if (gru && (!al16(d->hs[l]) || d->ldh % 8 || (d->h0[l] && (!al16(d->h0[l]) || d->ldh0 % 8)))) vec = false;
    if (d->dh_last[l] && !al16(d->dh_last[l])) vec = false;
    if (d->dh0[l] && !al16(d->dh0[l])) vec = false;
  }
  if (d->dy_a && (!pipe || dt != MVAE_BF16 || (long)B * d->dy_a_ld * sz >= (1L << 31) || (long)H * d->dy_w_ld * sz >= (1L << 31))) return MVAE_ERR_UNSUPPORTED;
  const int split_knob = tune_int("MVAE_BWD_SPLIT", 1);
  int nsplit = 0;
  if (split_knob && dt == MVAE_BF16 && pipe && vec && B % 128 == 0 && H % 128 == 0 && d->split_ws) {
    struct Cand { int bm, bn, ns, key; };
    static const Cand cand[7] = {{256, 128, 1, 2561}, {128, 128, 1, 1281}, {128, 64, 1, 641}, {256, 128, 2, 2562}, {128, 128, 2, 2}, {128, 128, 4, 1284}, {128, 64, 4, 644}};
    for (int c = 0; c < 7 && !nsplit; ++c) {
      if (B % cand[c].bm || (cand[c].ns == 4 && (4 * H) % (2 * ke))) continue;
      if (drop && cand[c].ns == 1) continue;
      const long wgs = (long)(B / cand[c].bm) * (H / cand[c].bn) * cand[c].ns * NL;
      if (split_knob == cand[c].key || (split_knob == 1 && wgs >= (cand[c].ns == 1 ? 256 : 192))) { BM = cand[c].bm; BN = cand[c].bn; nsplit = cand[c].ns; }
    }
    if (!nsplit && split_knob == 1 && (4 * H) % (2 * ke) == 0 && (long)(B / 128) * (H / 64) * 4 * NL >= 64) { BM = 128; BN = 64; nsplit = 4; }
    if (nsplit > 1 && d->split_ws_bytes < (size_t)NL * nsplit * B * H * sizeof(float)) { nsplit = 0; BM = 64; BN = 64; }
    if (split_knob == 1 && nsplit > 1) {
      const long fused_tiles = (long)((B + 63) / 64) * ((H + 63) / 64) * NL;
      const long kcols = (gru ? 6L : 8L) * H;
      if (fused_tiles >= 192 && 128 * kcols * sz <= (1L << 20)) { nsplit = 0; BM = 64; BN = 64; }
      if (NL == 1 && 128 * kcols * sz <= (1L << 20)) { nsplit = 0; BM = 64; BN = 64; }
    }
  }
  const bool big_fused = nsplit == 1;
  if (big_fused) nsplit = 0;
  const bool split = nsplit != 0;
  StepArgsB a;
  a.lengths = d->lengths; a.cell = d->cell; a.split = nsplit; a.partial = split ? reinterpret_cast<float*>(d->split_ws) : nullptr;
  a.drop.scale = drop ? 1.f / (1.f - d->drop_p) : 1.f;
  a.drop.thresh = drop ? (uint32_t)((double)d->drop_p * 4294967296.0) : 0u;
  a.drop.seed = d->drop_seed;
  a.gru3 = (gru && H % ke == 0 && (nsplit != 4 || (3 * H / 2) % ke == 0)) ? 1 : 0;
  a.B = B; a.H = H; a.tiles_m = (B + BM - 1) / BM; a.tiles_n = (H + BN - 1) / BN; a.vec = vec ? 1 : 0;
#ifdef MVAE_TUNING
  a.dbg = tune_int("MVAE_DBG", 0);
#else
  a.dbg = 0;
#endif
  const int nbuf = pipe ? (drop ? 4 : tune_int("MVAE_NBUF_BWD", 4)) : 0;
  size_t lds = (size_t)(split ? (BM == 256 ? 3 : 4) : big_fused ? (BM == 256 ? 3 : 4) : (nbuf > 0 ? nbuf : 2)) * (BM + BN) * KB;
  const size_t stage_bytes = (size_t)BM * (BN + 4) * sizeof(float);
  if (lds < stage_bytes) lds = stage_bytes;
  bool want_dh0 = false;
  for (int l = 0; l < NL; ++l) want_dh0 = want_dh0 || (gru && d->dh0[l]);
  for (int e = T + NL - 2; e >= (want_dh0 ? -1 : 0); --e) {
    int n = 0;
    if (e < 0) {
      for (int l = 0; l < NL; ++l) {
        if (!d->dh0[l]) continue;
        StepTaskB& q = a.t[n++];
        q.A0 = d->dG[l]; q.lda0 = ldg; q.K0 = 4 * H; q.W0 = d->w_hhT[l]; q.ldw0 = d->ldw_hhT[l];
        q.A1 = nullptr; q.lda1 = ldg; q.K1 = 4 * H; q.W1 = nullptr; q.ldw1 = 0;
        q.dy = nullptr; q.dy_ld = 0; q.gates = nullptr; q.c = nullptr; q.c_prev = nullptr;
        q.dc_in = d->dstate[l]; q.dc_out = nullptr; q.dG = nullptr; q.ldg = ldg; q.h_prev = nullptr; q.ldhp = 0;
        q.dh0 = d->dh0[l]; q.t = -1; q.drop = 0; q.dmask = nullptr; q.didx0 = 0; q.seg1_full = 0;
      }
      if (n == 0) break;
    }
    for (int l = 0; l < NL && e >= 0; ++l) {
      const int t = e - l;
      if (t < 0 || t >= T) continue;
      StepTaskB& q = a.t[n++];
      q.A0 = (t < T - 1) ? adv(d->dG[l], (long)(t + 1) * B * ldg, dt) : nullptr;
      q.lda0 = ldg; q.K0 = 4 * H; q.W0 = d->w_hhT[l]; q.ldw0 = d->ldw_hhT[l];
      q.A1 = (l < NL - 1) ? adv(d->dG[l + 1], (long)t * B * ldg, dt) : nullptr;
      q.lda1 = ldg; q.K1 = 4 * H; q.W1 = (l < NL - 1) ? d->w_ihT[l + 1] : nullptr; q.ldw1 = (l < NL - 1) ? d->ldw_ihT[l + 1] : 0;
      q.seg1_full = 0;
      if (l == NL - 1 && d->dy_a) {
        q.A1 = adv(d->dy_a, (long)t * B * d->dy_a_ld, dt); q.lda1 = d->dy_a_ld; q.K1 = d->dy_k; q.W1 = d->dy_w; q.ldw1 = d->dy_w_ld;
        q.seg1_full = 1;
      }
      q.dy = (l == NL - 1 && d->dy) ? d->dy + (long)t * B * d->dy_ld : nullptr; q.dy_ld = d->dy_ld;
      q.gates = adv(d->gates[l], (long)t * B * 4 * H, dt);
      q.c = gru ? nullptr : adv(d->cs[l], (long)t * B * H, dt);
      q.c_prev = (!gru && t > 0) ? adv(d->cs[l], (long)(t - 1) * B * H, dt) : nullptr;
      q.dc_in = (t < T - 1) ? d->dstate[l] + (long)((t + 1) & 1) * B * H : (gru ? d->dh_last[l] : nullptr);
      q.h_prev = gru ? ((t > 0) ? adv(d->hs[l], (long)(t - 1) * B * d->ldh, dt) : d->h0[l]) : nullptr;
      q.ldhp = (t > 0) ? d->ldh : d->ldh0;
      q.dh0 = nullptr; q.t = t;
      q.drop = (drop && l < NL - 1) ? 1 : 0;
      q.dmask = (q.drop && d->drop_mask[l]) ? d->drop_mask[l] + ((long)t * B) * H : nullptr;
      q.didx0 = (uint32_t)((((long)l * T + t) * B) * H);
      q.dc_out = d->dstate[l] + (long)(t & 1) * B * H;
      q.dG = const_cast<char*>(adv(d->dG[l], (long)t * B * ldg, dt)); q.ldg = ldg;
    }
    a.ntask = n;
    dim3 grid(n * a.tiles_m * a.tiles_n * (split ? nsplit : 1)), block(256);
    if (big_fused && drop) return MVAE_ERR_UNSUPPORTED;
    if (big_fused) {
      block = dim3(512);
      if (BM == 256) {
        MVAE_STEP_LAUNCH((lstm_step_bwd_kernel<bf16_t, 256, 128, 3, true, false, 0>));
        continue;
      }
      if (BN == 64) {
        if (d->dy) MVAE_STEP_LAUNCH((lstm_step_bwd_kernel<bf16_t, 128, 64, 4, true, false, 0, 1>));
        else MVAE_STEP_LAUNCH((lstm_step_bwd_kernel<bf16_t, 128, 64, 4, true, false, 0, 2>));
        continue;
      }
      if (d->dy) MVAE_STEP_LAUNCH((lstm_step_bwd_kernel<bf16_t, 128, 128, 4, true, false, 0, 1>));
      else MVAE_STEP_LAUNCH((lstm_step_bwd_kernel<bf16_t, 128, 128, 4, true, false, 0, 2>));
      continue;
    }
    if (split) {
      if (BM == 256) { block = dim3(512); MVAE_STEP_LAUNCH((lstm_step_bwd_kernel<bf16_t, 256, 128, 3, true, false, 1>)); block = dim3(256); }
      else if (BN == 64) { block = dim3(512); MVAE_STEP_LAUNCH((lstm_step_bwd_kernel<bf16_t, 128, 64, 4, true, false, 1>)); block = dim3(256); }
      else { block = dim3(512); MVAE_STEP_LAUNCH((lstm_step_bwd_kernel<bf16_t, 128, 128, 4, true, false, 1>)); block = dim3(256); }
      const long groups = (long)n * B * (H / 8);
      hipLaunchKernelGGL((lstm_bwd_epi_kernel<bf16_t>), dim3((unsigned)((groups + 255) / 256)), block, 0, st, a);
      continue;
    }
#define BWD_DROP(TT_, BM_, NB_) if (BM == BM_ && nbuf == NB_) { MVAE_STEP_LAUNCH((lstm_step_bwd_kernel<TT_, BM_, (BM_ == 32 ? 32 : 64), NB_, false, true>)); continue; }
    if (drop) {
      if (dt == MVAE_BF16) { BWD_DROP(bf16_t, 64, 4) BWD_DROP(bf16_t, 64, 0) }
      else { BWD_DROP(float, 64, 4) BWD_DROP(float, 64, 0) BWD_DROP(float, 32, 4) BWD_DROP(float, 32, 0) }
      return MVAE_ERR_UNSUPPORTED;
    }
#undef BWD_DROP
#define BWD_CASE(TT_, BM_, NB_) if (BM == BM_ && nbuf == NB_) { MVAE_STEP_LAUNCH((lstm_step_bwd_kernel<TT_, BM_, (BM_ == 32 ? 32 : 64), NB_>)); continue; }
    if (dt == MVAE_BF16) {
      BWD_CASE(bf16_t, 128, 0) BWD_CASE(bf16_t, 128, 3) BWD_CASE(bf16_t, 128, 4) BWD_CASE(bf16_t, 128, 5) BWD_CASE(bf16_t, 128, 6)
      BWD_CASE(bf16_t, 64, 0) BWD_CASE(bf16_t, 64, 3) BWD_CASE(bf16_t, 64, 4) BWD_CASE(bf16_t, 64, 5) BWD_CASE(bf16_t, 64, 6)
    } else {
      BWD_CASE(float, 128, 0) BWD_CASE(float, 128, 4) BWD_CASE(float, 64, 0) BWD_CASE(float, 64, 4) BWD_CASE(float, 32, 0) BWD_CASE(float, 32, 4)
    }
#undef BWD_CASE
    return MVAE_ERR_UNSUPPORTED;
  }
  MVAE_CHECK_HIP(hipGetLastError());
  return MVAE_OK;
}
```

### molecular-vae_amd/csrc/tile_pipe.hpp

```cpp
#pragma once
#include <type_traits>
#include "tile.hpp"

constexpr uint32_t PIPE_OOB = 0x80000000u;

template <int BM, int BN, int NT = 256> struct PipeSeg {
  __amdgpu_buffer_rsrc_t ra, rb;
  uint32_t offA[BM * 8 / NT];
  uint32_t offB[BN * 8 / NT];
  int nk;
  int hole_st; uint32_t hole_bytes;
};

template <typename T, int BM, int BN, int NT = 256, typename RowOffA, typename RowOffB>
__device__ __forceinline__ void pipe_seg_init(PipeSeg<BM, BN, NT>& s, const void* A, uint32_t bytesA, const void* B, uint32_t bytesB,
                                              RowOffA rowoffA, RowOffB rowoffB, int K, int tid) {
  constexpr int KE = KB / (int)sizeof(T);
  s.ra = __builtin_amdgcn_make_buffer_rsrc(const_cast<void*>(A), 0, (int)bytesA, 0x00020000);
  s.rb = __builtin_amdgcn_make_buffer_rsrc(const_cast<void*>(B), 0, (int)bytesB, 0x00020000);
  s.nk = (A != nullptr) ? K / KE : 0;
  s.hole_st = 0x7fffffff; s.hole_bytes = 0;
#pragma unroll
  for (int i = 0; i < BM * 8 / NT; ++i) {
    const int id = tid + i * NT, row = id >> 3, pos = id & 7;
    const uint32_t ro = rowoffA(row);
    s.offA[i] = (ro == PIPE_OOB) ? PIPE_OOB : ro + (uint32_t)(((pos ^ row) & 7) << 4);
  }
#pragma unroll
  for (int i = 0; i < BN * 8 / NT; ++i) {
    const int id = tid + i * NT, row = id >> 3, pos = id & 7;
    const uint32_t ro = rowoffB(row);
    s.offB[i] = (ro == PIPE_OOB) ? PIPE_OOB : ro + (uint32_t)(((pos ^ row) & 7) << 4);
  }
}

template <int N> __device__ __forceinline__ void wait_vmcnt() {
  static_assert(N >= 0 && N < 64, "vmcnt immediate");
  asm volatile("s_waitcnt vmcnt(%0)" ::"n"(N) : "memory");
}

typedef __attribute__((address_space(3))) void lds_void_t;

typedef __attribute__((ext_vector_type(4))) uint32_t u32x4;

template <int OFF> __device__ __forceinline__ u32x4 lds_read128(uint32_t addr) {
  u32x4 v;
  asm volatile("ds_read_b128 %0, %1 offset:%2" : "=v"(v) : "v"(addr), "n"(OFF));
  return v;
}
template <int I, int N, int STRIDE> struct FragRead {
  static __device__ __forceinline__ void run(u32x4 (&dst)[N], uint32_t addr) {
    dst[I] = lds_read128<I * STRIDE>(addr);
    FragRead<I + 1, N, STRIDE>::run(dst, addr);
  }
};
template <int N, int STRIDE> struct FragRead<N, N, STRIDE> {
  static __device__ __forceinline__ void run(u32x4 (&)[N], uint32_t) {}
};
template <int I, int N, int JS, int BOUT> struct FragReadB {
  static __device__ __forceinline__ void run(u32x4 (&dst)[N], uint32_t addr) {
    dst[I] = lds_read128<((I / JS) * BOUT + (I % JS) * 16) * KB>(addr);
    FragReadB<I + 1, N, JS, BOUT>::run(dst, addr);
  }
};
template <int N, int JS, int BOUT> struct FragReadB<N, N, JS, BOUT> {
  static __device__ __forceinline__ void run(u32x4 (&)[N], uint32_t) {}
};
template <int N> __device__ __forceinline__ void wait_lgkmcnt() {
  __builtin_amdgcn_sched_barrier(0);
  asm volatile("s_waitcnt lgkmcnt(%0)" ::"n"(N) : "memory");
  __builtin_amdgcn_sched_barrier(0);
}

__device__ __forceinline__ void split_x3(const u32x4& c0, const u32x4& c1, uint4& hi, uint4& lo) {
  const uint32_t x[8] = {c0[0], c0[1], c0[2], c0[3], c1[0], c1[1], c1[2], c1[3]};
  uint32_t h[4], l[4];
#pragma unroll
  for (int j = 0; j < 4; ++j) {
    const uint32_t h0 = x[2 * j] & 0xffff0000u, h1 = x[2 * j + 1] & 0xffff0000u;
    const float l0 = __builtin_bit_cast(float, x[2 * j]) - __builtin_bit_cast(float, h0);
    const float l1 = __builtin_bit_cast(float, x[2 * j + 1]) - __builtin_bit_cast(float, h1);
    h[j] = (h0 >> 16) | h1;
    l[j] = (uint32_t)f2bf(l0) | ((uint32_t)f2bf(l1) << 16);
  }
  hi = make_uint4(h[0], h[1], h[2], h[3]); lo = make_uint4(l[0], l[1], l[2], l[3]);
}
template <int MI, int NI, int JS, int BOUT>
__device__ __forceinline__ void tile_mma_asm_x3(uint32_t a_base, uint32_t b_base, const uint32_t (&a_lane)[2], const uint32_t (&b_lane)[2],
                                                f32x4 (&acc)[MI][NI]) {
  u32x4 a0[MI], b0[NI], a1[MI], b1[NI];
  FragRead<0, MI, 16 * KB>::run(a0, a_base + a_lane[0]);
  FragReadB<0, NI, JS, BOUT>::run(b0, b_base + b_lane[0]);
  FragRead<0, MI, 16 * KB>::run(a1, a_base + a_lane[1]);
  FragReadB<0, NI, JS, BOUT>::run(b1, b_base + b_lane[1]);
  wait_lgkmcnt<0>();
  uint4 ah[MI], al[MI], bh[NI], bl[NI];
#pragma unroll
  for (int mi = 0; mi < MI; ++mi) split_x3(a0[mi], a1[mi], ah[mi], al[mi]);
#pragma unroll
  for (int ni = 0; ni < NI; ++ni) split_x3(b0[ni], b1[ni], bh[ni], bl[ni]);
#pragma unroll
  for (int mi = 0; mi < MI; ++mi)
#pragma unroll
    for (int ni = 0; ni < NI; ++ni) {
      mma16<bf16_t>(al[mi], bh[ni], acc[mi][ni]);
      mma16<bf16_t>(ah[mi], bl[ni], acc[mi][ni]);
      mma16<bf16_t>(ah[mi], bh[ni], acc[mi][ni]);
    }
}

template <typename T, int MI, int NI, int JS, int BOUT>
__device__ __forceinline__ void tile_mma_asm(uint32_t a_base, uint32_t b_base, const uint32_t (&a_lane)[2], const uint32_t (&b_lane)[2],
                                             f32x4 (&acc)[MI][NI]) {
  u32x4 a0[MI], b0[NI], a1[MI], b1[NI];
  FragRead<0, MI, 16 * KB>::run(a0, a_base + a_lane[0]);
  FragReadB<0, NI, JS, BOUT>::run(b0, b_base + b_lane[0]);
  FragRead<0, MI, 16 * KB>::run(a1, a_base + a_lane[1]);
  FragReadB<0, NI, JS, BOUT>::run(b1, b_base + b_lane[1]);
  wait_lgkmcnt<(MI + NI) < 16 ? (MI + NI) : 15>();
#pragma unroll
  for (int mi = 0; mi < MI; ++mi)
#pragma unroll
    for (int ni = 0; ni < NI; ++ni)
      mma16<T>(__builtin_bit_cast(uint4, a0[mi]), __builtin_bit_cast(uint4, b0[ni]), acc[mi][ni]);
  wait_lgkmcnt<0>();
#pragma unroll
  for (int mi = 0; mi < MI; ++mi)
#pragma unroll
    for (int ni = 0; ni < NI; ++ni)
      mma16<T>(__builtin_bit_cast(uint4, a1[mi]), __builtin_bit_cast(uint4, b1[ni]), acc[mi][ni]);
}

__device__ __forceinline__ void ws_barrier() {
  __builtin_amdgcn_sched_barrier(0);
  __builtin_amdgcn_s_barrier();
  asm volatile("" ::: "memory");
  __builtin_amdgcn_sched_barrier(0);
}

template <int BM, int BN, int NBUF, int NT = 256>
__device__ __forceinline__ void pipe_issue_stage(char* smem, const PipeSeg<BM, BN, NT>& s0, const PipeSeg<BM, BN, NT>& s1, int st, int wave) {
#if defined(__HIP_DEVICE_COMPILE__)
  char* stage = smem + (st % NBUF) * ((BM + BN) * KB);
  const bool first = st < s0.nk;
  const PipeSeg<BM, BN, NT>& s = first ? s0 : s1;
  const int ls = first ? st : st - s0.nk;
  const uint32_t kbyte = (uint32_t)ls * KB + (ls >= s.hole_st ? s.hole_bytes : 0u);
#pragma unroll
  for (int i = 0; i < BM * 8 / NT; ++i) {
    lds_void_t* dst = (lds_void_t*)(stage + (i * NT + wave * 64) * 16);
    __builtin_amdgcn_raw_ptr_buffer_load_lds(s.ra, dst, 16, s.offA[i] + kbyte, 0, 0, 0);
  }
#pragma unroll
  for (int i = 0; i < BN * 8 / NT; ++i) {
    lds_void_t* dst = (lds_void_t*)(stage + BM * KB + (i * NT + wave * 64) * 16);
    __builtin_amdgcn_raw_ptr_buffer_load_lds(s.rb, dst, 16, s.offB[i] + kbyte, 0, 0, 0);
  }
#endif
}

template <typename T, int BM, int BN, int MI, int NI, int NBUF, int JS, int BOUT, bool X3 = false>
__device__ __forceinline__ void tile_gemm_pipe(char* smem, const PipeSeg<BM, BN>& s0, const PipeSeg<BM, BN>& s1, int arow0,
                                               int brow0, f32x4 (&acc)[MI][NI], int tid) {
  static_assert(!X3 || std::is_same<T, float>::value, "the 3 x bf16 product form takes fp32 operands");
  constexpr int STAGE = (BM + BN) * KB;
  constexpr int LPS = (BM + BN) * 8 / 256;
  static_assert((NBUF - 2) * LPS < 64, "vmcnt range");
  static_assert((BM + BN) * 8 % 256 == 0 && BM * 8 % 256 == 0, "whole LDS-DMA pieces per thread");
  const int lane = tid & 63;
  const int wave = __builtin_amdgcn_readfirstlane(tid >> 6);
  const int nk = s0.nk + s1.nk;
  if (nk <= 0) return;
  const uint32_t lds0 = (uint32_t)(uintptr_t)(lds_void_t*)smem;
  const int lr = lane & 15, lk = lane >> 4;
  uint32_t a_lane[2], b_lane[2];
#pragma unroll
  for (int kk = 0; kk < 2; ++kk) {
    a_lane[kk] = (uint32_t)swz(arow0 + lr, kk * 4 + lk);
    b_lane[kk] = (uint32_t)swz(brow0 + lr, kk * 4 + lk) + BM * KB;
  }
#pragma unroll
  for (int s = 0; s < NBUF - 1; ++s)
    if (s < nk) pipe_issue_stage<BM, BN, NBUF>(smem, s0, s1, s, wave);
  for (int kt = 0; kt < nk; ++kt) {
    if (kt + NBUF - 2 < nk) wait_vmcnt<(NBUF - 2) * LPS>();
    else wait_vmcnt<0>();
    __builtin_amdgcn_s_barrier();
    asm volatile("" ::: "memory");
    if (kt + NBUF - 1 < nk) pipe_issue_stage<BM, BN, NBUF>(smem, s0, s1, kt + NBUF - 1, wave);
    const uint32_t st = lds0 + (uint32_t)((kt % NBUF) * STAGE);
    if constexpr (X3) tile_mma_asm_x3<MI, NI, JS, BOUT>(st, st, a_lane, b_lane, acc);
    else tile_mma_asm<T, MI, NI, JS, BOUT>(st, st, a_lane, b_lane, acc);
  }
  __builtin_amdgcn_s_barrier();
}


__device__ __forceinline__ void SB() { __builtin_amdgcn_sched_barrier(0); }

template <typename T, int MI, int NI, int M0, int M1>
__device__ __forceinline__ void mma_rows(const u32x4 (&a)[MI], const u32x4 (&b)[NI], f32x4 (&acc)[MI][NI]) {
#pragma unroll
  for (int mi = M0; mi < M1; ++mi)
#pragma unroll
    for (int ni = 0; ni < NI; ++ni)
      mma16<T>(__builtin_bit_cast(uint4, a[mi]), __builtin_bit_cast(uint4, b[ni]), acc[mi][ni]);
}

template <typename T, int BM, int BN, int NBUF, int NT, int MI, int NI, int GA, int M0>
__device__ __forceinline__ void pipe_block_with_refill(char* smem, const PipeSeg<BM, BN, NT>& s0, const PipeSeg<BM, BN, NT>& s1, bool refill, int st,
                                                       int wave, const u32x4 (&a)[GA], const u32x4 (&b)[NI], f32x4 (&acc)[MI][NI]) {
  if (refill) pipe_issue_stage<BM, BN, NBUF, NT>(smem, s0, s1, st, wave);
  SB();
#pragma unroll
  for (int r = 0; r < GA; ++r)
#pragma unroll
    for (int ni = 0; ni < NI; ++ni) mma16<T>(__builtin_bit_cast(uint4, a[r]), __builtin_bit_cast(uint4, b[ni]), acc[M0 + r][ni]);
}
template <typename T, int MI, int NI, int GA, int M0>
__device__ __forceinline__ void pipe_block(const u32x4 (&a)[GA], const u32x4 (&b)[NI], f32x4 (&acc)[MI][NI]) {
#pragma unroll
  for (int r = 0; r < GA; ++r)
#pragma unroll
    for (int ni = 0; ni < NI; ++ni) mma16<T>(__builtin_bit_cast(uint4, a[r]), __builtin_bit_cast(uint4, b[ni]), acc[M0 + r][ni]);
}

template <typename T, int BM, int BN, int MI, int NI, int NBUF, int NT>
__device__ __forceinline__ void tile_gemm_pipe_all(char* smem, const PipeSeg<BM, BN, NT>& s0, const PipeSeg<BM, BN, NT>& s1, int arow0,
                                                   int brow0, f32x4 (&acc)[MI][NI], int tid) {
  constexpr int STAGE = (BM + BN) * KB;
  constexpr int LPS = (BM + BN) * 8 / NT;
  constexpr int GA = MI / 2;
  constexpr bool STAGGER = NT == 512;
  static_assert(MI % 2 == 0 && NBUF >= 2 && (NBUF - 2) * LPS < 64, "vmcnt range");
  static_assert(GA + NI <= 15, "lgkmcnt range");
  static_assert(BM * 8 % NT == 0 && BN * 8 % NT == 0, "whole LDS-DMA pieces per thread");
  const int lane = tid & 63;
  const int wave = __builtin_amdgcn_readfirstlane(tid >> 6);
  const bool late = STAGGER && wave >= NT / 128;
  const int nk = s0.nk + s1.nk;
  if (nk <= 0) return;
  const uint32_t lds0 = (uint32_t)(uintptr_t)(lds_void_t*)smem;
  const int lr = lane & 15, lk = lane >> 4;
  uint32_t a_lane[2], b_lane[2];
#pragma unroll
  for (int kk = 0; kk < 2; ++kk) {
    a_lane[kk] = (uint32_t)swz(arow0 + lr, kk * 4 + lk);
    b_lane[kk] = (uint32_t)swz(brow0 + lr, kk * 4 + lk) + BM * KB;
  }
  constexpr uint32_t G1 = GA * 16 * KB;
#pragma unroll
  for (int s = 0; s < NBUF - 1; ++s)
    if (s < nk) pipe_issue_stage<BM, BN, NBUF, NT>(smem, s0, s1, s, wave);
  u32x4 aX[GA], aY[GA], bh0[NI], bh1[NI];
  if (NBUF - 2 < nk) wait_vmcnt<(NBUF - 2) * LPS>(); else wait_vmcnt<0>();
  ws_barrier();
  int pend = (NBUF - 1 < nk) ? NBUF - 1 : -1;
  if (pend >= 0 && !late) { pipe_issue_stage<BM, BN, NBUF, NT>(smem, s0, s1, pend, wave); pend = -1; }
  FragRead<0, GA, 16 * KB>::run(aX, lds0 + a_lane[0]);
  FragReadB<0, NI, NI, 0>::run(bh0, lds0 + b_lane[0]);
  for (int kt = 0; kt < nk; ++kt) {
    const uint32_t st = lds0 + (uint32_t)((kt % NBUF) * STAGE);
    FragRead<0, GA, 16 * KB>::run(aY, st + a_lane[0] + G1);
    FragReadB<0, NI, NI, 0>::run(bh1, st + b_lane[1]);
    wait_lgkmcnt<GA + NI>();
    if constexpr (STAGGER) {
      pipe_block_with_refill<T, BM, BN, NBUF, NT, MI, NI, GA, 0>(smem, s0, s1, late && pend >= 0, pend, wave, aX, bh0, acc);
      if (late) pend = -1;
    } else pipe_block<T, MI, NI, GA, 0>(aX, bh0, acc);
    SB();
    FragRead<0, GA, 16 * KB>::run(aX, st + a_lane[1]);
    wait_lgkmcnt<NI + GA>();
    pipe_block<T, MI, NI, GA, GA>(aY, bh0, acc);
    SB();
    FragRead<0, GA, 16 * KB>::run(aY, st + a_lane[1] + G1);
    wait_lgkmcnt<GA>();
    pipe_block<T, MI, NI, GA, 0>(aX, bh1, acc);
    wait_lgkmcnt<0>();
    if (kt + 1 < nk) {
      if (kt + 1 + NBUF - 2 < nk) wait_vmcnt<(NBUF - 2) * LPS>(); else wait_vmcnt<0>();
      ws_barrier();
      pend = (kt + NBUF < nk) ? kt + NBUF : -1;
      const uint32_t sn = lds0 + (uint32_t)(((kt + 1) % NBUF) * STAGE);
      FragRead<0, GA, 16 * KB>::run(aX, sn + a_lane[0]);
      FragReadB<0, NI, NI, 0>::run(bh0, sn + b_lane[0]);
    }
    pipe_block_with_refill<T, BM, BN, NBUF, NT, MI, NI, GA, GA>(smem, s0, s1, !late && pend >= 0, pend, wave, aY, bh1, acc);
    if (!late) pend = -1;
    SB();
  }
}

typedef __attribute__((ext_vector_type(2))) uint32_t u32x2;

template <int OFF> __device__ __forceinline__ u32x2 lds_read_tr64(uint32_t addr) {
  u32x2 v;
  asm volatile("ds_read_b64_tr_b16 %0, %1 offset:%2" : "=v"(v) : "v"(addr), "n"(OFF));
  return v;
}

template <int MI> struct PipeSegTN {
  __amdgpu_buffer_rsrc_t ra, rb;
  uint32_t offA[MI], offB[4];
  uint32_t kstepA, kstepB;
  int nk;
};

__device__ __forceinline__ uint32_t tn_f(int krow) { return (uint32_t)((krow & 3) | (((krow >> 3) & 1) << 2)); }

template <int MI>
__device__ __forceinline__ void pipe_seg_tn_init(PipeSegTN<MI>& s, const void* A, long lda, int m0, const void* B, long ldb, int n0,
                                                 int K, int tid) {
#if defined(__HIP_DEVICE_COMPILE__)
  constexpr int RA = 64 * MI;
  constexpr int RPP = 1024 / RA;
  constexpr int CPR = RA / 16;
  s.ra = __builtin_amdgcn_make_buffer_rsrc(const_cast<void*>(A), 0, (int)((long)K * lda * 2), 0x00020000);
  s.rb = __builtin_amdgcn_make_buffer_rsrc(const_cast<void*>(B), 0, (int)((long)K * ldb * 2), 0x00020000);
  s.nk = (K + 63) / 64;
  s.kstepA = (uint32_t)(64 * lda * 2);
  s.kstepB = (uint32_t)(64 * ldb * 2);
  const int wave = tid >> 6, lane = tid & 63;
#pragma unroll
  for (int i = 0; i < MI; ++i) {
    const int ii = i * 4 + wave;
    const int krow = ii * RPP + lane / CPR, pc = lane % CPR;
    const uint32_t lc = (uint32_t)((((pc >> 1) ^ tn_f(krow)) << 1) | (pc & 1));
    s.offA[i] = (uint32_t)krow * (uint32_t)(lda * 2) + (uint32_t)(m0 * 2) + lc * 16u;
  }
#pragma unroll
  for (int i = 0; i < 4; ++i) {
    const int ii = i * 4 + wave;
    const int krow = ii * 4 + (lane >> 4), pc = lane & 15;
    const uint32_t lc = (uint32_t)((((pc >> 1) ^ tn_f(krow)) << 1) | (pc & 1));
    s.offB[i] = (uint32_t)krow * (uint32_t)(ldb * 2) + (uint32_t)(n0 * 2) + lc * 16u;
  }
#endif
}

template <int NBUF, int MI>
__device__ __forceinline__ void pipe_tn_issue(char* smem, const PipeSegTN<MI>& s, int st, int wave) {
#if defined(__HIP_DEVICE_COMPILE__)
  constexpr int ABYTES = 64 * 64 * MI, STAGE = ABYTES + 16384;
  char* stage = smem + (st % NBUF) * STAGE;
#pragma unroll
  for (int i = 0; i < MI; ++i) {
    lds_void_t* dst = (lds_void_t*)(stage + (i * 4 + wave) * 1024);
    __builtin_amdgcn_raw_ptr_buffer_load_lds(s.ra, dst, 16, s.offA[i] + (uint32_t)st * s.kstepA, 0, 0, 0);
  }
#pragma unroll
  for (int i = 0; i < 4; ++i) {
    lds_void_t* dst = (lds_void_t*)(stage + ABYTES + (i * 4 + wave) * 1024);
    __builtin_amdgcn_raw_ptr_buffer_load_lds(s.rb, dst, 16, s.offB[i] + (uint32_t)st * s.kstepB, 0, 0, 0);
  }
#endif
}

template <int I, int N, int ROWB> struct FragReadTN {
  template <int KOFF>
  static __device__ __forceinline__ void run(u32x4 (&dst)[N], const uint32_t (&addr)[N], uint32_t st) {
    const u32x2 lo = lds_read_tr64<KOFF>(st + addr[I]);
    const u32x2 hi = lds_read_tr64<KOFF + 4 * ROWB>(st + addr[I]);
    dst[I] = u32x4{lo[0], lo[1], hi[0], hi[1]};
    FragReadTN<I + 1, N, ROWB>::template run<KOFF>(dst, addr, st);
  }
};
template <int N, int ROWB> struct FragReadTN<N, N, ROWB> {
  template <int KOFF> static __device__ __forceinline__ void run(u32x4 (&)[N], const uint32_t (&)[N], uint32_t) {}
};

template <int NBUF, int MI>
__device__ __forceinline__ void tile_gemm_ws_tn(char* smem, const PipeSegTN<MI>& s, int wm, int wn, f32x4 (&acc)[MI][4], int tid) {
  constexpr int LPS = MI + 4;
  constexpr int RA = 64 * MI, ABYTES = 64 * RA, STAGE = ABYTES + 16384;
  static_assert((NBUF - 2) * LPS < 64, "vmcnt range");
  const int lane = tid & 63;
  const int wave = __builtin_amdgcn_readfirstlane(tid >> 6);
  const int nk = s.nk;
  if (nk <= 0) return;
  if (wave >= 4) {
#pragma unroll
    for (int st = 0; st < NBUF - 1; ++st)
      if (st < nk) pipe_tn_issue<NBUF, MI>(smem, s, st, wave - 4);
    for (int kt = 0; kt < nk; ++kt) {
      if (kt + NBUF - 2 < nk) wait_vmcnt<(NBUF - 2) * LPS>();
      else wait_vmcnt<0>();
      ws_barrier();
      if (kt + NBUF - 1 < nk) pipe_tn_issue<NBUF, MI>(smem, s, kt + NBUF - 1, wave - 4);
    }
  } else {
    const uint32_t lds0 = (uint32_t)(uintptr_t)(lds_void_t*)smem;
    const int g = lane >> 4, q = (lane >> 2) & 3, pp = lane & 3;
    const uint32_t f = (uint32_t)(q | ((g & 1) << 2));
    uint32_t addrA[MI], addrB[4];
#pragma unroll
    for (int i = 0; i < MI; ++i) addrA[i] = (uint32_t)(8 * g + q) * (uint32_t)RA + ((((uint32_t)(wm * MI + i)) ^ f) << 5) + (uint32_t)pp * 8u;
#pragma unroll
    for (int i = 0; i < 4; ++i) addrB[i] = (uint32_t)(8 * g + q) * 256u + ((((uint32_t)(wn * 4 + i)) ^ f) << 5) + (uint32_t)pp * 8u + (uint32_t)ABYTES;
    u32x4 a0[MI], b0[4], a1[MI], b1[4];
    ws_barrier();
    FragReadTN<0, MI, RA>::template run<0>(a0, addrA, lds0);
    FragReadTN<0, 4, 256>::template run<0>(b0, addrB, lds0);
    for (int kt = 0; kt < nk; ++kt) {
      const uint32_t st = lds0 + (uint32_t)((kt % NBUF) * STAGE);
      wait_lgkmcnt<0>();
      FragReadTN<0, MI, RA>::template run<32 * RA>(a1, addrA, st);
      FragReadTN<0, 4, 256>::template run<32 * 256>(b1, addrB, st);
#pragma unroll
      for (int mi = 0; mi < MI; ++mi)
#pragma unroll
        for (int ni = 0; ni < 4; ++ni)
          mma16<bf16_t>(__builtin_bit_cast(uint4, a0[mi]), __builtin_bit_cast(uint4, b0[ni]), acc[mi][ni]);
      wait_lgkmcnt<0>();
      if (kt + 1 < nk) {
        ws_barrier();
        const uint32_t sn = lds0 + (uint32_t)(((kt + 1) % NBUF) * STAGE);
        FragReadTN<0, MI, RA>::template run<0>(a0, addrA, sn);
        FragReadTN<0, 4, 256>::template run<0>(b0, addrB, sn);
      }
#pragma unroll
      for (int mi = 0; mi < MI; ++mi)
#pragma unroll
        for (int ni = 0; ni < 4; ++ni)
          mma16<bf16_t>(__builtin_bit_cast(uint4, a1[mi]), __builtin_bit_cast(uint4, b1[ni]), acc[mi][ni]);
    }
  }
  ws_barrier();
}

template <int MI, int NI, int JS, int BOUT, int R>
__device__ __forceinline__ void ilv_read(u32x4 (&na)[MI], u32x4 (&nb)[NI], uint32_t a_addr, uint32_t b_addr) {
  if constexpr (R == 0) na[0] = lds_read128<0>(a_addr);
  else if constexpr (R <= NI) nb[R - 1] = lds_read128<(((R - 1) / JS) * BOUT + ((R - 1) % JS) * 16) * KB>(b_addr);
  else if constexpr (R < MI + NI) na[R - NI] = lds_read128<(R - NI) * 16 * KB>(a_addr);
}
template <typename T, int MI, int NI, int JS, int BOUT, int M, bool RD = true> struct MmaIlv {
  static constexpr int RPG = (MI + NI + MI * NI - 1) / (MI * NI);
  static __device__ __forceinline__ void run(const u32x4 (&a)[MI], const u32x4 (&b)[NI], f32x4 (&acc)[MI][NI], u32x4 (&na)[MI], u32x4 (&nb)[NI],
                                             uint32_t a_addr, uint32_t b_addr) {
    constexpr int mi = M / NI, ni = M % NI;
    mma16<T>(__builtin_bit_cast(uint4, a[mi]), __builtin_bit_cast(uint4, b[ni]), acc[mi][ni]);
    if constexpr (RD && M * RPG < MI + NI) {
      __builtin_amdgcn_sched_barrier(0);
      ilv_read<MI, NI, JS, BOUT, M * RPG>(na, nb, a_addr, b_addr);
      if constexpr (RPG > 1) ilv_read<MI, NI, JS, BOUT, M * RPG + 1>(na, nb, a_addr, b_addr);
      static_assert(RPG <= 2, "at most two reads per gap");
      __builtin_amdgcn_sched_barrier(0);
    }
    MmaIlv<T, MI, NI, JS, BOUT, M + 1, RD>::run(a, b, acc, na, nb, a_addr, b_addr);
  }
};
template <typename T, int MI, int NI, int JS, int BOUT, bool RD> struct MmaIlv<T, MI, NI, JS, BOUT, MI * NI, RD> {
  static __device__ __forceinline__ void run(const u32x4 (&)[MI], const u32x4 (&)[NI], f32x4 (&)[MI][NI], u32x4 (&)[MI], u32x4 (&)[NI], uint32_t, uint32_t) {}
};

template <typename T, int BM, int BN, int NBUF>
__device__ __forceinline__ void tile_gemm_ws_loader(char* smem, const PipeSeg<BM, BN>& s0, const PipeSeg<BM, BN>& s1, int lwave, int dbg = 0) {
  constexpr int LPS = (BM + BN) * 8 / 256;
  static_assert((NBUF - 2) * LPS < 64, "vmcnt range");
  const int nk = s0.nk + s1.nk;
#ifdef MVAE_TUNING
  const bool issue = !(dbg & 8);
#else
  constexpr bool issue = true;
#endif
#pragma unroll
  for (int s = 0; s < NBUF - 1; ++s)
    if (s < nk && issue) pipe_issue_stage<BM, BN, NBUF>(smem, s0, s1, s, lwave);
  for (int kt = 0; kt < nk; ++kt) {
    if (kt + NBUF - 2 < nk) wait_vmcnt<(NBUF - 2) * LPS>();
    else wait_vmcnt<0>();
    ws_barrier();
    if (kt + NBUF - 1 < nk && issue) pipe_issue_stage<BM, BN, NBUF>(smem, s0, s1, kt + NBUF - 1, lwave);
  }
}
template <typename T, int BM, int BN, int NBUF, int NTAIL, typename Tail>
__device__ __forceinline__ void tile_gemm_ws_loader_tail(char* smem, const PipeSeg<BM, BN>& s0, const PipeSeg<BM, BN>& s1, int lwave, Tail tail) {
  constexpr int LPS = (BM + BN) * 8 / 256;
  static_assert((NBUF - 2) * LPS + NTAIL < 64, "vmcnt range");
  static_assert(NBUF == 4, "tail waits written out for a ring of four");
  const int nk = s0.nk + s1.nk;
#pragma unroll
  for (int s = 0; s < NBUF - 1; ++s) pipe_issue_stage<BM, BN, NBUF>(smem, s0, s1, s, lwave);
  for (int kt = 0; kt <= nk - NBUF; ++kt) {
    wait_vmcnt<(NBUF - 2) * LPS>();
    ws_barrier();
    pipe_issue_stage<BM, BN, NBUF>(smem, s0, s1, kt + NBUF - 1, lwave);
  }
  __builtin_amdgcn_sched_barrier(0);
  asm volatile("" ::: "memory");
  tail();
  asm volatile("" ::: "memory");
  __builtin_amdgcn_sched_barrier(0);
  wait_vmcnt<2 * LPS + NTAIL>(); ws_barrier();
  wait_vmcnt<1 * LPS + NTAIL>(); ws_barrier();
  wait_vmcnt<NTAIL>(); ws_barrier();
}
template <typename T, int BM, int BN, int MI, int NI, int NBUF, int JS, int BOUT, bool ILV = false>
__device__ __forceinline__ void tile_gemm_ws_consumer(char* smem, int nk, int arow0, int brow0, f32x4 (&acc)[MI][NI], int lane, int dbg = 0) {
#ifdef MVAE_TUNING
  const bool do_mma = !(dbg & 16), do_rd = !(dbg & 32);
#else
  constexpr bool do_mma = true, do_rd = true;
#endif
  constexpr int STAGE = (BM + BN) * KB;
  static_assert(MI + NI <= 15, "lgkmcnt range");
  const uint32_t lds0 = (uint32_t)(uintptr_t)(lds_void_t*)smem;
  const int lr = lane & 15, lk = lane >> 4;
  uint32_t a_lane[2], b_lane[2];
#pragma unroll
  for (int kk = 0; kk < 2; ++kk) {
    a_lane[kk] = (uint32_t)swz(arow0 + lr, kk * 4 + lk);
    b_lane[kk] = (uint32_t)swz(brow0 + lr, kk * 4 + lk) + BM * KB;
  }
  u32x4 a0[MI], b0[NI], a1[MI], b1[NI];
  ws_barrier();
  if (ILV && do_mma && do_rd) {
  FragRead<0, MI, 16 * KB>::run(a0, lds0 + a_lane[0]);
  FragReadB<0, NI, JS, BOUT>::run(b0, lds0 + b_lane[0]);
  wait_lgkmcnt<0>();
  for (int kt = 0; kt < nk; ++kt) {
    const uint32_t st = lds0 + (uint32_t)((kt % NBUF) * STAGE);
    MmaIlv<T, MI, NI, JS, BOUT, 0>::run(a0, b0, acc, a1, b1, st + a_lane[1], st + b_lane[1]);
    wait_lgkmcnt<0>();
    if (kt + 1 < nk) {
      ws_barrier();
      const uint32_t sn = lds0 + (uint32_t)(((kt + 1) % NBUF) * STAGE);
      MmaIlv<T, MI, NI, JS, BOUT, 0>::run(a1, b1, acc, a0, b0, sn + a_lane[0], sn + b_lane[0]);
      wait_lgkmcnt<0>();
    } else {
      MmaIlv<T, MI, NI, JS, BOUT, 0, false>::run(a1, b1, acc, a0, b0, 0u, 0u);
    }
  }
  } else {
  if (do_rd) {
  FragRead<0, MI, 16 * KB>::run(a0, lds0 + a_lane[0]);
  FragReadB<0, NI, JS, BOUT>::run(b0, lds0 + b_lane[0]);
  }
  for (int kt = 0; kt < nk; ++kt) {
    const uint32_t st = lds0 + (uint32_t)((kt % NBUF) * STAGE);
    if (do_rd) {
    FragRead<0, MI, 16 * KB>::run(a1, st + a_lane[1]);
    FragReadB<0, NI, JS, BOUT>::run(b1, st + b_lane[1]);
    }
    wait_lgkmcnt<MI + NI>();
    if (do_mma) {
#pragma unroll
    for (int mi = 0; mi < MI; ++mi)
#pragma unroll
      for (int ni = 0; ni < NI; ++ni)
        mma16<T>(__builtin_bit_cast(uint4, a0[mi]), __builtin_bit_cast(uint4, b0[ni]), acc[mi][ni]);
    }
    wait_lgkmcnt<0>();
    if (kt + 1 < nk) {
      ws_barrier();
      const uint32_t sn = lds0 + (uint32_t)(((kt + 1) % NBUF) * STAGE);
      if (do_rd) {
      FragRead<0, MI, 16 * KB>::run(a0, sn + a_lane[0]);
      FragReadB<0, NI, JS, BOUT>::run(b0, sn + b_lane[0]);
      }
    }
    if (do_mma) {
#pragma unroll
    for (int mi = 0; mi < MI; ++mi)
#pragma unroll
      for (int ni = 0; ni < NI; ++ni)
        mma16<T>(__builtin_bit_cast(uint4, a1[mi]), __builtin_bit_cast(uint4, b1[ni]), acc[mi][ni]);
    }
  }
  }
}

template <typename T, int BM, int BN, int MI, int NI, int NBUF, int JS, int BOUT, bool ILV = false>
__device__ __forceinline__ void tile_gemm_ws(char* smem, const PipeSeg<BM, BN>& s0, const PipeSeg<BM, BN>& s1, int arow0, int brow0,
                                             f32x4 (&acc)[MI][NI], int tid) {
  const int lane = tid & 63;
  const int wave = __builtin_amdgcn_readfirstlane(tid >> 6);
  const int nk = s0.nk + s1.nk;
  if (nk <= 0) return;
  if (wave >= 4) tile_gemm_ws_loader<T, BM, BN, NBUF>(smem, s0, s1, wave - 4);
  else tile_gemm_ws_consumer<T, BM, BN, MI, NI, NBUF, JS, BOUT, ILV>(smem, nk, arow0, brow0, acc, lane);
  ws_barrier();
}

struct PipeSegTN2 {
  __amdgpu_buffer_rsrc_t ra, rb;
  uint32_t offA[4], offB[4];
  uint32_t kstepA, kstepB;
  int nk;
};

__device__ __forceinline__ void pipe_seg_tn2_init(PipeSegTN2& s, const void* A, long lda, int m0, const void* B, long ldb, int n0, int K, int tid) {
#if defined(__HIP_DEVICE_COMPILE__)
  s.ra = __builtin_amdgcn_make_buffer_rsrc(const_cast<void*>(A), 0, (int)((long)K * lda * 2), 0x00020000);
  s.rb = __builtin_amdgcn_make_buffer_rsrc(const_cast<void*>(B), 0, (int)((long)K * ldb * 2), 0x00020000);
  s.nk = (K + 63) / 64;
  s.kstepA = (uint32_t)(64 * lda * 2);
  s.kstepB = (uint32_t)(64 * ldb * 2);
  const int wave = tid >> 6, lane = tid & 63;
#pragma unroll
  for (int i = 0; i < 4; ++i) {
    const int ii = i * 8 + wave;
    const int krow = ii * 2 + (lane >> 5), pc = lane & 31;
    const uint32_t lc = (uint32_t)((((pc >> 1) ^ tn_f(krow)) << 1) | (pc & 1));
    s.offA[i] = (uint32_t)krow * (uint32_t)(lda * 2) + (uint32_t)(m0 * 2) + lc * 16u;
    s.offB[i] = (uint32_t)krow * (uint32_t)(ldb * 2) + (uint32_t)(n0 * 2) + lc * 16u;
  }
#endif
}

__device__ __forceinline__ void pipe_tn2_issue(char* smem, const PipeSegTN2& s, int st, int wave) {
#if defined(__HIP_DEVICE_COMPILE__)
  char* stage = smem + (st & 1) * 65536;
#pragma unroll
  for (int i = 0; i < 4; ++i) {
    lds_void_t* dst = (lds_void_t*)(stage + (i * 8 + wave) * 1024);
    __builtin_amdgcn_raw_ptr_buffer_load_lds(s.ra, dst, 16, s.offA[i] + (uint32_t)st * s.kstepA, 0, 0, 0);
  }
#pragma unroll
  for (int i = 0; i < 4; ++i) {
    lds_void_t* dst = (lds_void_t*)(stage + 32768 + (i * 8 + wave) * 1024);
    __builtin_amdgcn_raw_ptr_buffer_load_lds(s.rb, dst, 16, s.offB[i] + (uint32_t)st * s.kstepB, 0, 0, 0);
  }
#endif
}

template <int M> struct TnIlv {
  static __device__ __forceinline__ void run(const u32x4 (&a0)[8], const u32x4 (&b0)[4], f32x4 (&acc)[8][4], u32x2 (&lo)[12], u32x2 (&hi)[12],
                                             const uint32_t (&addrA)[8], const uint32_t (&addrB)[4], uint32_t st) {
    constexpr int mi = M / 4, ni = M % 4;
    mma16<bf16_t>(__builtin_bit_cast(uint4, a0[mi]), __builtin_bit_cast(uint4, b0[ni]), acc[mi][ni]);
    if constexpr (M < 24) {
      constexpr int F = M >> 1;
      __builtin_amdgcn_sched_barrier(0);
      const uint32_t ad = st + (F < 8 ? addrA[F < 8 ? F : 0] : addrB[F < 8 ? 0 : F - 8]);
      if constexpr ((M & 1) == 0) lo[F] = lds_read_tr64<32 * 512>(ad);
      else hi[F] = lds_read_tr64<32 * 512 + 4 * 512>(ad);
      __builtin_amdgcn_sched_barrier(0);
    }
    TnIlv<M + 1>::run(a0, b0, acc, lo, hi, addrA, addrB, st);
  }
};
template <> struct TnIlv<32> {
  static __device__ __forceinline__ void run(const u32x4 (&)[8], const u32x4 (&)[4], f32x4 (&)[8][4], u32x2 (&)[12], u32x2 (&)[12], const uint32_t (&)[8],
                                             const uint32_t (&)[4], uint32_t) {}
};
template <bool COLSUM>
__device__ __forceinline__ void tile_gemm_tn_256(char* smem, const PipeSegTN2& s, int wm, int wn, f32x4 (&acc)[8][4], int cs_mi, int cs_half, f32x4& accb,
                                                 int tid) {
  const int lane = tid & 63;
  const int wave = __builtin_amdgcn_readfirstlane(tid >> 6);
  const int nk = s.nk;
  if (nk <= 0) return;
  const uint32_t lds0 = (uint32_t)(uintptr_t)(lds_void_t*)smem;
  const int g = lane >> 4, q = (lane >> 2) & 3, pp = lane & 3;
  const uint32_t f = (uint32_t)(q | ((g & 1) << 2));
  uint32_t addrA[8], addrB[4];
#pragma unroll
  for (int i = 0; i < 8; ++i) addrA[i] = (uint32_t)(8 * g + q) * 512u + ((((uint32_t)(wm * 8 + i)) ^ f) << 5) + (uint32_t)pp * 8u;
#pragma unroll
  for (int i = 0; i < 4; ++i) addrB[i] = (uint32_t)(8 * g + q) * 512u + ((((uint32_t)(wn * 4 + i)) ^ f) << 5) + (uint32_t)pp * 8u + 32768u;
  const uint4 ones = make_uint4(0x3F803F80u, 0x3F803F80u, 0x3F803F80u, 0x3F803F80u);
  uint32_t addrS[1];
  addrS[0] = (uint32_t)(8 * g + q) * 512u + ((((uint32_t)(wm * 8 + (cs_mi & 7))) ^ f) << 5) + (uint32_t)pp * 8u + (cs_half == 1 ? 32u * 512u : 0u);
  pipe_tn2_issue(smem, s, 0, wave);
  for (int kt = 0; kt < nk; ++kt) {
    wait_vmcnt<0>();
    ws_barrier();
    const uint32_t st = lds0 + (uint32_t)((kt & 1) * 65536);
    u32x4 a0[8], b0[4], a1[8], b1[4], as[1];
    u32x2 lo[12], hi[12];
    FragReadTN<0, 8, 512>::template run<0>(a0, addrA, st);
    FragReadTN<0, 4, 512>::template run<0>(b0, addrB, st);
    if constexpr (COLSUM) FragReadTN<0, 1, 512>::template run<0>(as, addrS, st);
    __builtin_amdgcn_sched_barrier(0);
    asm volatile("" ::: "memory");
    if (kt + 1 < nk) pipe_tn2_issue(smem, s, kt + 1, wave);
    wait_lgkmcnt<0>();
    TnIlv<0>::run(a0, b0, acc, lo, hi, addrA, addrB, st);
    if constexpr (COLSUM) {
      if (cs_half >= 0) mma16<bf16_t>(__builtin_bit_cast(uint4, as[0]), ones, accb);
    }
    wait_lgkmcnt<0>();
#pragma unroll
    for (int i = 0; i < 8; ++i) a1[i] = u32x4{lo[i][0], lo[i][1], hi[i][0], hi[i][1]};
#pragma unroll
    for (int i = 0; i < 4; ++i) b1[i] = u32x4{lo[8 + i][0], lo[8 + i][1], hi[8 + i][0], hi[8 + i][1]};
#pragma unroll
    for (int mi = 0; mi < 8; ++mi)
#pragma unroll
      for (int ni = 0; ni < 4; ++ni)
        mma16<bf16_t>(__builtin_bit_cast(uint4, a1[mi]), __builtin_bit_cast(uint4, b1[ni]), acc[mi][ni]);
  }
  ws_barrier();
}
```

Baseline: 36590.

## Add persistent ticket-scheduled LSTM forward kernel for the 256x256 GEMM tile path

Adds a persistent LSTM forward kernel for the 256x256 tile configuration. One workgroup per CU pulls (layer, timestep, row-block, tile) tickets from an atomic counter and spins on per-tile done counters, so it no longer launches one step kernel per timestep and layer. The shared tile body is moved into a header and reused by both the per-step and persistent kernels. It also adds a cache-policy (aux) template parameter to the LDS-DMA buffer loads, presumably to control coherence of the B loads. The cost is spin-wait dependency tracking, a workspace memset per launch, and the risk of stalls or deadlock if the ticket order does not match dependency readiness.

Result: slower. 35930 (median of 2 runs) (-1.8%).

```diff
diff --git a/molecular-vae_amd/csrc/capi.hip b/molecular-vae_amd/csrc/capi.hip
--- a/molecular-vae_amd/csrc/capi.hip
+++ b/molecular-vae_amd/csrc/capi.hip
@@ -89,6 +89,7 @@
 size_t mvae_rnn_fwd_persist_workspace(const mvae_rnn_fwd_desc* d) {
   if (!d) return 0;
   if (rnn_persist_fwd_supported(d)) return rnn_persist_fwd_workspace_bytes(d->T);
+  if (rnn_persist_gm_fwd_supported(d)) return rnn_persist_gm_fwd_workspace_bytes(d);
   return rnn_rowres_fwd_pipe_workspace(d);
 }
 int mvae_rnn_bwd(const mvae_rnn_bwd_desc* d, void* stream, const void** status_out) {
diff --git a/molecular-vae_amd/csrc/kernels.hpp b/molecular-vae_amd/csrc/kernels.hpp
--- a/molecular-vae_amd/csrc/kernels.hpp
+++ b/molecular-vae_amd/csrc/kernels.hpp
@@ -34,6 +34,9 @@
 bool rnn_persist_fwd_supported(const mvae_rnn_fwd_desc* d);
 size_t rnn_persist_fwd_workspace_bytes(int T);
 int rnn_persist_fwd(const mvae_rnn_fwd_desc* d, void* ws, size_t ws_bytes, hipStream_t st);
+bool rnn_persist_gm_fwd_supported(const mvae_rnn_fwd_desc* d);
+size_t rnn_persist_gm_fwd_workspace_bytes(const mvae_rnn_fwd_desc* d);
+int rnn_persist_gm_fwd(const mvae_rnn_fwd_desc* d, void* ws, size_t ws_bytes, hipStream_t st);
 bool rnn_persist_bwd_supported(const mvae_rnn_bwd_desc* d);
 size_t rnn_persist_bwd_workspace_bytes(int T);
 int rnn_persist_bwd(const mvae_rnn_bwd_desc* d, void* ws, size_t ws_bytes, hipStream_t st);
diff --git a/molecular-vae_amd/csrc/rnn.hip b/molecular-vae_amd/csrc/rnn.hip
--- a/molecular-vae_amd/csrc/rnn.hip
+++ b/molecular-vae_amd/csrc/rnn.hip
@@ -1,29 +1,8 @@
 #include "tile_pipe.hpp"
 #include "kernels.hpp"
+#include "rnn_gm.hpp"
 #include <stdlib.h>
 
-template <typename T> __device__ __forceinline__ void load8(const T* p, float (&v)[8]);
-template <> __device__ __forceinline__ void load8<float>(const float* p, float (&v)[8]) {
-  const float4 a = *reinterpret_cast<const float4*>(p), b = *reinterpret_cast<const float4*>(p + 4);
-  v[0] = a.x; v[1] = a.y; v[2] = a.z; v[3] = a.w; v[4] = b.x; v[5] = b.y; v[6] = b.z; v[7] = b.w;
-}
-template <> __device__ __forceinline__ void load8<bf16_t>(const bf16_t* p, float (&v)[8]) {
-  const uint4 u = *reinterpret_cast<const uint4*>(p);
-  const uint32_t w[4] = {u.x, u.y, u.z, u.w};
-#pragma unroll
-  for (int i = 0; i < 4; ++i) { v[2 * i] = __builtin_bit_cast(float, w[i] << 16); v[2 * i + 1] = __builtin_bit_cast(float, w[i] & 0xffff0000u); }
-}
-template <typename T> __device__ __forceinline__ void store8(T* p, const float (&v)[8]);
-template <> __device__ __forceinline__ void store8<float>(float* p, const float (&v)[8]) {
-  *reinterpret_cast<float4*>(p) = make_float4(v[0], v[1], v[2], v[3]);
-  *reinterpret_cast<float4*>(p + 4) = make_float4(v[4], v[5], v[6], v[7]);
-}
-template <> __device__ __forceinline__ void store8<bf16_t>(bf16_t* p, const float (&v)[8]) {
-  uint4 u;
-  u.x = (uint32_t)f2bf(v[0]) | ((uint32_t)f2bf(v[1]) << 16); u.y = (uint32_t)f2bf(v[2]) | ((uint32_t)f2bf(v[3]) << 16);
-  u.z = (uint32_t)f2bf(v[4]) | ((uint32_t)f2bf(v[5]) << 16); u.w = (uint32_t)f2bf(v[6]) | ((uint32_t)f2bf(v[7]) << 16);
-  *reinterpret_cast<uint4*>(p) = u;
-}
 template <typename T> __device__ __forceinline__ void ldn(const T* p, float (&v)[8], int n, bool vec) {
   if (vec && n == 8) { load8<T>(p, v); return; }
 #pragma unroll
@@ -34,13 +13,6 @@
 #pragma unroll
   for (int e = 0; e < 8; ++e) if (e < n) TT<T>::st(p + e, v[e]);
 }
-
-template <typename T> __device__ __forceinline__ float act_sigmoid(float x);
-template <typename T> __device__ __forceinline__ float act_tanh(float x);
-template <> __device__ __forceinline__ float act_sigmoid<float>(float x) { return 1.f / (1.f + expf(-x)); }
-template <> __device__ __forceinline__ float act_tanh<float>(float x) { return tanhf(x); }
-template <> __device__ __forceinline__ float act_sigmoid<bf16_t>(float x) { return __builtin_amdgcn_rcpf(1.f + __expf(-x)); }
-template <> __device__ __forceinline__ float act_tanh<bf16_t>(float x) { return fmaf(-2.f, __builtin_amdgcn_rcpf(1.f + __expf(2.f * x)), 1.f); }
 
 __device__ __forceinline__ int xcd_remap_r(int bid, int n) {
   const int q = n >> 3, r = n & 7, x = bid & 7, i = bid >> 3;
@@ -58,24 +30,6 @@
   return keep ? da.scale : 0.f;
 }
 
-struct StepTaskF {
-  const void *A0, *A1, *W0, *W1;
-  long lda0, lda1, ldw0, ldw1;
-  int K0, K1;
-  const float* add; long add_ld;
-  const float* add_tbl;
-  const int64_t* add_idx; long add_idx_ld; int add_rows;
-  const float* bias;
-  const float* c_prev; float* c_out;
-  void* c_save;
-  void* h_out; long ldh;
-  void* g_out;
-  const void* hprev_t0;
-  int t;
-  void* h_drop;
-  const uint8_t* dmask;
-  uint32_t didx0;
-};
 struct StepArgsF { StepTaskF t[MVAE_MAX_LAYERS]; const int* lengths; int ntask, B, H, tiles_m, tiles_j, dbg, vec, cell, gru3; DropArgs drop; };
 
 template <typename T, int BM, int BJ, int NBUF, bool WS = false>
@@ -319,162 +273,16 @@
   else { if (has_add) rows(std::false_type{}, std::true_type{}); else rows(std::false_type{}, std::false_type{}); }
 }
 
+
 template <int BMW, int BNB, int NBUF, bool WS = false>
 __global__ __launch_bounds__(WS ? 512 : BMW * 2) void lstm_step_fwd_gm_kernel(StepArgsF p) {
-  using T = bf16_t;
   extern __shared__ __attribute__((aligned(16))) char smem[];
-  static_assert(BMW == 256 || BMW == 128, "weight rows per tile: 64 or 32 units x 4 gates");
-  static_assert(!WS || BMW == 128, "loader / consumer split: the 4-wave tile only");
-  constexpr int NT = BMW * 2;
-  constexpr int BU = BMW / 4;
-  constexpr int MI = 8, NI = BNB / 64;
-  const int tid = threadIdx.x, lane = tid & 63, wave = WS ? ((tid >> 6) & 3) : (tid >> 6), wm = wave >> 2, wn = wave & 3;
   const int per_task = p.tiles_m * p.tiles_j;
   const int bid = xcd_remap_r(blockIdx.x, p.ntask * per_task);
   const int task = bid / per_task;
   const int rem = bid - task * per_task;
   const int tj = rem / p.tiles_m, tm = rem - tj * p.tiles_m;
-  const StepTaskF& q = p.t[task];
-  const int n0 = tm * BNB, j0 = tj * BU, H = p.H, B = p.B;
-
-  const int lq = lane >> 4, lc = lane & 15;
-  const int ub = j0 + 32 * wm + 8 * lq;
-  constexpr bool BIAS_FIRST = (BMW == 256 && BNB == 256);
-  auto load_bias = [&](float (&bias)[4][8]) {
-    if (q.bias) {
-#pragma unroll
-      for (int g = 0; g < 4; ++g) load8<float>(q.bias + g * H + ub, bias[g]);
-    } else {
-#pragma unroll
-      for (int g = 0; g < 4; ++g)
-#pragma unroll
-        for (int e = 0; e < 8; ++e) bias[g][e] = 0.f;
-    }
-  };
-  f32x4 acc[MI][NI];
-  if constexpr (BIAS_FIRST) {
-    float bias[4][8];
-    load_bias(bias);
-#pragma unroll
-    for (int ni = 0; ni < NI; ++ni)
-#pragma unroll
-      for (int g = 0; g < 4; ++g)
-#pragma unroll
-        for (int e = 0; e < 8; ++e) acc[2 * g + (e >> 2)][ni][e & 3] = bias[g][e];
-  } else {
-#pragma unroll
-    for (int i = 0; i < MI; ++i)
-#pragma unroll
-      for (int g = 0; g < NI; ++g) acc[i][g] = f32x4{0.f, 0.f, 0.f, 0.f};
-  }
-
-  float cpa[NI][8];
-  auto load_cprev_all = [&]() {
-    const float* cpsrc = q.c_prev ? q.c_prev : q.c_out;
-#pragma unroll
-    for (int ni = 0; ni < NI; ++ni) {
-      const int row = n0 + wn * (16 * NI) + ni * 16 + lc;
-      load8<float>(cpsrc + (long)(row < B ? row : B - 1) * H + ub, cpa[ni]);
-    }
-  };
-  if constexpr (BIAS_FIRST) load_cprev_all();
-
-#ifdef MVAE_TUNING
-  const bool run_main = !(p.dbg & 2);
-#else
-  constexpr bool run_main = true;
-#endif
-  if (run_main) {
-    PipeSeg<BMW, BNB, NT> s0, s1;
-    auto wrow = [&](int r) -> int {
-      const int mi = (r >> 4) & 7, j = r & 15;
-      return (mi >> 1) * H + j0 + 32 * (r >> 7) + 8 * (j >> 2) + 4 * (mi & 1) + (j & 3);
-    };
-    {
-      const uint32_t lda = (uint32_t)q.lda0 * 2u, ldw = (uint32_t)q.ldw0 * 2u;
-      auto offW = [&](int r) -> uint32_t { return (uint32_t)wrow(r) * ldw; };
-      auto offX = [&](int r) -> uint32_t { const int gn = n0 + r; return gn < B ? (uint32_t)gn * lda : PIPE_OOB; };
-      pipe_seg_init<T, BMW, BNB, NT>(s0, q.W0, (uint32_t)(4 * H) * ldw, q.A0, (uint32_t)B * lda, offW, offX, q.K0, WS ? (tid & 255) : tid);
-      if (q.A0 == nullptr) s0.nk = 0;
-    }
-    {
-      const uint32_t lda = (uint32_t)q.lda1 * 2u, ldw = (uint32_t)q.ldw1 * 2u;
-      auto offW = [&](int r) -> uint32_t { return (uint32_t)wrow(r) * ldw; };
-      auto offX = [&](int r) -> uint32_t { const int gn = n0 + r; return gn < B ? (uint32_t)gn * lda : PIPE_OOB; };
-      pipe_seg_init<T, BMW, BNB, NT>(s1, q.W1, (uint32_t)(4 * H) * ldw, q.A1, (uint32_t)B * lda, offW, offX, q.K1, WS ? (tid & 255) : tid);
-      if (q.A1 == nullptr) s1.nk = 0;
-    }
-    if constexpr (WS) tile_gemm_ws<T, BMW, BNB, MI, NI, NBUF, NI, 0>(smem, s0, s1, 0, wn * (16 * NI), acc, tid);
-    else tile_gemm_pipe_all<T, BMW, BNB, MI, NI, NBUF, NT>(smem, s0, s1, wm * 128, wn * (16 * NI), acc, tid);
-  }
-  if constexpr (WS) { if (tid >= 256) return; }
-#ifdef MVAE_TUNING
-  if (p.dbg & 1) { if (acc[0][0][0] == 12345.678f) q.c_out[0] = 1.f; return; }
-#endif
-
-  if constexpr (!BIAS_FIRST) {
-    float bias[4][8];
-    load_bias(bias);
-#pragma unroll
-    for (int ni = 0; ni < NI; ++ni)
-#pragma unroll
-      for (int g = 0; g < 4; ++g)
-#pragma unroll
-        for (int e = 0; e < 8; ++e) acc[2 * g + (e >> 2)][ni][e & 3] += bias[g][e];
-  }
-  T* hout = reinterpret_cast<T*>(q.h_out);
-  T* gout = reinterpret_cast<T*>(q.g_out);
-  T* csave = reinterpret_cast<T*>(q.c_save);
-  if constexpr (!BIAS_FIRST) load_cprev_all();
-  const bool has_cprev = q.c_prev != nullptr;
-  auto epilogue = [&](auto has_add, auto full_tile) {
-#pragma unroll
-  for (int ni = 0; ni < NI; ++ni) {
-    const int row = n0 + wn * (16 * NI) + ni * 16 + lc;
-    if constexpr (!decltype(full_tile)::value) { if (row >= B) continue; }
-    float cp[8];
-#pragma unroll
-    for (int e = 0; e < 8; ++e) cp[e] = has_cprev ? cpa[ni][e] : 0.f;
-    float pre[4][8];
-#pragma unroll
-    for (int g = 0; g < 4; ++g)
-#pragma unroll
-      for (int e = 0; e < 8; ++e) pre[g][e] = acc[2 * g + (e >> 2)][ni][e & 3];
-    if constexpr (decltype(has_add)::value) {
-#pragma unroll
-      for (int g = 0; g < 4; ++g) {
-        float a[8];
-        load8<float>(q.add + (long)row * q.add_ld + g * H + ub, a);
-#pragma unroll
-        for (int e = 0; e < 8; ++e) pre[g][e] += a[e];
-      }
-    }
-    float gi[8], gf[8], gg[8], go[8], c[8], h[8];
-#pragma unroll
-    for (int e = 0; e < 8; ++e) {
-      gi[e] = act_sigmoid<T>(pre[0][e]); gf[e] = act_sigmoid<T>(pre[1][e]); gg[e] = act_tanh<T>(pre[2][e]); go[e] = act_sigmoid<T>(pre[3][e]);
-      c[e] = gf[e] * cp[e] + gi[e] * gg[e];
-      h[e] = go[e] * act_tanh<T>(c[e]);
-    }
-#ifdef MVAE_TUNING
-    const int srow = (p.dbg & 4) ? n0 + (row & 15) : row;
-    const bool sgate = !(p.dbg & 8);
-#else
-    const int srow = row;
-    constexpr bool sgate = true;
-#endif
-    store8<float>(q.c_out + (long)srow * H + ub, c);
-    store8<T>(hout + (long)srow * q.ldh + ub, h);
-    if (gout) {
-      T* g4 = gout + (long)srow * 4 * H + ub;
-      store8<T>(csave + (long)srow * H + ub, c);
-      if (sgate) { store8<T>(g4, gi); store8<T>(g4 + H, gf); store8<T>(g4 + 2 * H, gg); store8<T>(g4 + 3 * H, go); }
-    }
-  }
-  };
-  const bool full = n0 + BNB <= B;
-  if (q.add) { if (full) epilogue(std::true_type{}, std::true_type{}); else epilogue(std::true_type{}, std::false_type{}); }
-  else { if (full) epilogue(std::false_type{}, std::true_type{}); else epilogue(std::false_type{}, std::false_type{}); }
+  lstm_fwd_gm_tile<BMW, BNB, NBUF, WS, false>(p.t[task], p.B, p.H, p.dbg, tm, tj, smem, [] {});
 }
 
 struct StepTaskB {
@@ -1135,6 +943,8 @@
     }
   }
   if (BMW) { BM = BNB; BJ = BMW / 4; }
+  if (BMW == 256 && BNB == 256 && d->persist_ws && !d->no_spin && rnn_persist_gm_fwd_supported(d))
+    return rnn_persist_gm_fwd(d, d->persist_ws, d->persist_ws_bytes, st);
   a.B = B; a.H = H; a.tiles_m = (B + BM - 1) / BM; a.tiles_j = (H + BJ - 1) / BJ; a.vec = vec ? 1 : 0;
   a.drop.scale = drop ? 1.f / (1.f - d->drop_p) : 1.f;
   a.drop.thresh = drop ? (uint32_t)((double)d->drop_p * 4294967296.0) : 0u;
diff --git a/molecular-vae_amd/csrc/rnn_gm.hpp b/molecular-vae_amd/csrc/rnn_gm.hpp
--- /dev/null
+++ b/molecular-vae_amd/csrc/rnn_gm.hpp
@@ -0,0 +1,255 @@
+#pragma once
+#include "tile_pipe.hpp"
+#include "kernels.hpp"
+
+template <typename T> __device__ __forceinline__ void load8(const T* p, float (&v)[8]);
+template <> __device__ __forceinline__ void load8<float>(const float* p, float (&v)[8]) {
+  const float4 a = *reinterpret_cast<const float4*>(p), b = *reinterpret_cast<const float4*>(p + 4);
+  v[0] = a.x; v[1] = a.y; v[2] = a.z; v[3] = a.w; v[4] = b.x; v[5] = b.y; v[6] = b.z; v[7] = b.w;
+}
+template <> __device__ __forceinline__ void load8<bf16_t>(const bf16_t* p, float (&v)[8]) {
+  const uint4 u = *reinterpret_cast<const uint4*>(p);
+  const uint32_t w[4] = {u.x, u.y, u.z, u.w};
+#pragma unroll
+  for (int i = 0; i < 4; ++i) { v[2 * i] = __builtin_bit_cast(float, w[i] << 16); v[2 * i + 1] = __builtin_bit_cast(float, w[i] & 0xffff0000u); }
+}
+template <typename T> __device__ __forceinline__ void store8(T* p, const float (&v)[8]);
+template <> __device__ __forceinline__ void store8<float>(float* p, const float (&v)[8]) {
+  *reinterpret_cast<float4*>(p) = make_float4(v[0], v[1], v[2], v[3]);
+  *reinterpret_cast<float4*>(p + 4) = make_float4(v[4], v[5], v[6], v[7]);
+}
+__device__ __forceinline__ uint4 pack8bf(const float (&v)[8]) {
+  uint4 u;
+  u.x = (uint32_t)f2bf(v[0]) | ((uint32_t)f2bf(v[1]) << 16); u.y = (uint32_t)f2bf(v[2]) | ((uint32_t)f2bf(v[3]) << 16);
+  u.z = (uint32_t)f2bf(v[4]) | ((uint32_t)f2bf(v[5]) << 16); u.w = (uint32_t)f2bf(v[6]) | ((uint32_t)f2bf(v[7]) << 16);
+  return u;
+}
+template <> __device__ __forceinline__ void store8<bf16_t>(bf16_t* p, const float (&v)[8]) { *reinterpret_cast<uint4*>(p) = pack8bf(v); }
+
+template <typename T> __device__ __forceinline__ float act_sigmoid(float x);
+template <typename T> __device__ __forceinline__ float act_tanh(float x);
+template <> __device__ __forceinline__ float act_sigmoid<float>(float x) { return 1.f / (1.f + expf(-x)); }
+template <> __device__ __forceinline__ float act_tanh<float>(float x) { return tanhf(x); }
+template <> __device__ __forceinline__ float act_sigmoid<bf16_t>(float x) { return __builtin_amdgcn_rcpf(1.f + __expf(-x)); }
+template <> __device__ __forceinline__ float act_tanh<bf16_t>(float x) { return fmaf(-2.f, __builtin_amdgcn_rcpf(1.f + __expf(2.f * x)), 1.f); }
+
+struct StepTaskF {
+  const void *A0, *A1, *W0, *W1;
+  long lda0, lda1, ldw0, ldw1;
+  int K0, K1;
+  const float* add; long add_ld;
+  const float* add_tbl;
+  const int64_t* add_idx; long add_idx_ld; int add_rows;
+  const float* bias;
+  const float* c_prev; float* c_out;
+  void* c_save;
+  void* h_out; long ldh;
+  void* g_out;
+  const void* hprev_t0;
+  int t;
+  void* h_drop;
+  const uint8_t* dmask;
+  uint32_t didx0;
+};
+
+template <int BMW, int BNB, int NBUF, bool WS, bool PERSIST, typename Publish>
+__device__ __forceinline__ void lstm_fwd_gm_tile(const StepTaskF& q, int B, int H, int dbg, int tm, int tj, char* smem, Publish&& publish) {
+  using T = bf16_t;
+  static_assert(BMW == 256 || BMW == 128, "weight rows per tile: 64 or 32 units x 4 gates");
+  static_assert(!WS || BMW == 128, "loader / consumer split: the 4-wave tile only");
+  static_assert(!PERSIST || (BMW == 256 && BNB == 256 && !WS), "persistent pass: the 256 x 256 tile only");
+  constexpr int NT = BMW * 2;
+  constexpr int BU = BMW / 4;
+  constexpr int MI = 8, NI = BNB / 64;
+  int tid = threadIdx.x;
+  if constexpr (PERSIST) asm volatile("" : "+v"(tid));
+  const int lane = tid & 63, wave = WS ? ((tid >> 6) & 3) : (tid >> 6), wm = wave >> 2, wn = wave & 3;
+  const int n0 = tm * BNB, j0 = tj * BU;
+  (void)dbg;
+  const int lq = lane >> 4, lc = lane & 15;
+  const int ub = j0 + 32 * wm + 8 * lq;
+  constexpr bool BIAS_FIRST = (BMW == 256 && BNB == 256);
+  auto load_bias = [&](float (&bias)[4][8]) {
+    if (q.bias) {
+#pragma unroll
+      for (int g = 0; g < 4; ++g) load8<float>(q.bias + g * H + ub, bias[g]);
+    } else {
+#pragma unroll
+      for (int g = 0; g < 4; ++g)
+#pragma unroll
+        for (int e = 0; e < 8; ++e) bias[g][e] = 0.f;
+    }
+  };
+  f32x4 acc[MI][NI];
+  if constexpr (BIAS_FIRST) {
+    float bias[4][8];
+    load_bias(bias);
+#pragma unroll
+    for (int ni = 0; ni < NI; ++ni)
+#pragma unroll
+      for (int g = 0; g < 4; ++g)
+#pragma unroll
+        for (int e = 0; e < 8; ++e) acc[2 * g + (e >> 2)][ni][e & 3] = bias[g][e];
+  } else {
+#pragma unroll
+    for (int i = 0; i < MI; ++i)
+#pragma unroll
+      for (int g = 0; g < NI; ++g) acc[i][g] = f32x4{0.f, 0.f, 0.f, 0.f};
+  }
+
+  float cpa[NI][8];
+  auto load_cprev_all = [&]() {
+    const float* cpsrc = q.c_prev ? q.c_prev : q.c_out;
+#pragma unroll
+    for (int ni = 0; ni < NI; ++ni) {
+      const int row = n0 + wn * (16 * NI) + ni * 16 + lc;
+      if constexpr (PERSIST) {
+        const __amdgpu_buffer_rsrc_t rc = __builtin_amdgcn_make_buffer_rsrc(const_cast<float*>(cpsrc), 0, B * H * 4, 0x00020000);
+        const uint32_t off = (uint32_t)((row * H + ub) * 4);
+        const f32x4 lo = __builtin_bit_cast(f32x4, __builtin_amdgcn_raw_buffer_load_b128(rc, off, 0, 16));
+        const f32x4 hi = __builtin_bit_cast(f32x4, __builtin_amdgcn_raw_buffer_load_b128(rc, off + 16, 0, 16));
+#pragma unroll
+        for (int e = 0; e < 4; ++e) { cpa[ni][e] = lo[e]; cpa[ni][4 + e] = hi[e]; }
+      } else {
+        load8<float>(cpsrc + (long)(row < B ? row : B - 1) * H + ub, cpa[ni]);
+      }
+    }
+  };
+  if constexpr (BIAS_FIRST) load_cprev_all();
+
+#ifdef MVAE_TUNING
+  const bool run_main = !(dbg & 2);
+#else
+  constexpr bool run_main = true;
+#endif
+  if (run_main) {
+    PipeSeg<BMW, BNB, NT> s0, s1;
+    auto wrow = [&](int r) -> int {
+      const int mi = (r >> 4) & 7, j = r & 15;
+      return (mi >> 1) * H + j0 + 32 * (r >> 7) + 8 * (j >> 2) + 4 * (mi & 1) + (j & 3);
+    };
+    {
+      const uint32_t lda = (uint32_t)q.lda0 * 2u, ldw = (uint32_t)q.ldw0 * 2u;
+      auto offW = [&](int r) -> uint32_t { return (uint32_t)wrow(r) * ldw; };
+      auto offX = [&](int r) -> uint32_t { const int gn = n0 + r; return gn < B ? (uint32_t)gn * lda : PIPE_OOB; };
+      pipe_seg_init<T, BMW, BNB, NT>(s0, q.W0, (uint32_t)(4 * H) * ldw, q.A0, (uint32_t)B * lda, offW, offX, q.K0, WS ? (tid & 255) : tid);
+      if (q.A0 == nullptr) s0.nk = 0;
+    }
+    {
+      const uint32_t lda = (uint32_t)q.lda1 * 2u, ldw = (uint32_t)q.ldw1 * 2u;
+      auto offW = [&](int r) -> uint32_t { return (uint32_t)wrow(r) * ldw; };
+      auto offX = [&](int r) -> uint32_t { const int gn = n0 + r; return gn < B ? (uint32_t)gn * lda : PIPE_OOB; };
+      pipe_seg_init<T, BMW, BNB, NT>(s1, q.W1, (uint32_t)(4 * H) * ldw, q.A1, (uint32_t)B * lda, offW, offX, q.K1, WS ? (tid & 255) : tid);
+      if (q.A1 == nullptr) s1.nk = 0;
+    }
+    if constexpr (WS) tile_gemm_ws<T, BMW, BNB, MI, NI, NBUF, NI, 0>(smem, s0, s1, 0, wn * (16 * NI), acc, tid);
+    else tile_gemm_pipe_all<T, BMW, BNB, MI, NI, NBUF, NT, PERSIST ? 16 : 0>(smem, s0, s1, wm * 128, wn * (16 * NI), acc, tid);
+  }
+  if constexpr (WS) { if (tid >= 256) return; }
+#ifdef MVAE_TUNING
+  if (dbg & 1) { if (acc[0][0][0] == 12345.678f) q.c_out[0] = 1.f; return; }
+#endif
+
+  if constexpr (!BIAS_FIRST) {
+    float bias[4][8];
+    load_bias(bias);
+#pragma unroll
+    for (int ni = 0; ni < NI; ++ni)
+#pragma unroll
+      for (int g = 0; g < 4; ++g)
+#pragma unroll
+        for (int e = 0; e < 8; ++e) acc[2 * g + (e >> 2)][ni][e & 3] += bias[g][e];
+  }
+  T* hout = reinterpret_cast<T*>(q.h_out);
+  T* gout = reinterpret_cast<T*>(q.g_out);
+  T* csave = reinterpret_cast<T*>(q.c_save);
+  if constexpr (!BIAS_FIRST) load_cprev_all();
+  const bool has_cprev = q.c_prev != nullptr;
+  [[maybe_unused]] uint4 c_park[NI];
+  const uint32_t park = (uint32_t)(uintptr_t)(lds_void_t*)smem + (uint32_t)(tid << 4);
+  auto epilogue = [&](auto has_add, auto full_tile) {
+#pragma unroll
+  for (int ni = 0; ni < NI; ++ni) {
+    const int row = n0 + wn * (16 * NI) + ni * 16 + lc;
+    if constexpr (!decltype(full_tile)::value) { if (row >= B) continue; }
+    float cp[8];
+#pragma unroll
+    for (int e = 0; e < 8; ++e) cp[e] = has_cprev ? cpa[ni][e] : 0.f;
+    float pre[4][8];
+#pragma unroll
+    for (int g = 0; g < 4; ++g)
+#pragma unroll
+      for (int e = 0; e < 8; ++e) pre[g][e] = acc[2 * g + (e >> 2)][ni][e & 3];
+    if constexpr (decltype(has_add)::value) {
+#pragma unroll
+      for (int g = 0; g < 4; ++g) {
+        float a[8];
+        load8<float>(q.add + (long)row * q.add_ld + g * H + ub, a);
+#pragma unroll
+        for (int e = 0; e < 8; ++e) pre[g][e] += a[e];
+      }
+    }
+    float gi[8], gf[8], gg[8], go[8], c[8], h[8];
+#pragma unroll
+    for (int e = 0; e < 8; ++e) {
+      gi[e] = act_sigmoid<T>(pre[0][e]); gf[e] = act_sigmoid<T>(pre[1][e]); gg[e] = act_tanh<T>(pre[2][e]); go[e] = act_sigmoid<T>(pre[3][e]);
+      c[e] = fmaf(gf[e], cp[e], gi[e] * gg[e]);
+      h[e] = go[e] * act_tanh<T>(c[e]);
+    }
+#ifdef MVAE_TUNING
+    const int srow = (dbg & 4) ? n0 + (row & 15) : row;
+    const bool sgate = !(dbg & 8);
+#else
+    const int srow = row;
+    constexpr bool sgate = true;
+#endif
+    if constexpr (PERSIST) {
+      const __amdgpu_buffer_rsrc_t rc = __builtin_amdgcn_make_buffer_rsrc(q.c_out, 0, B * H * 4, 0x00020000);
+      const __amdgpu_buffer_rsrc_t rh = __builtin_amdgcn_make_buffer_rsrc(hout, 0, (int)((long)B * q.ldh * 2), 0x00020000);
+      const uint32_t coff = (uint32_t)((srow * H + ub) * 4);
+      __builtin_amdgcn_raw_buffer_store_b128(__builtin_bit_cast(u32x4, f32x4{c[0], c[1], c[2], c[3]}), rc, coff, 0, 17);
+      __builtin_amdgcn_raw_buffer_store_b128(__builtin_bit_cast(u32x4, f32x4{c[4], c[5], c[6], c[7]}), rc, coff + 16, 0, 17);
+      __builtin_amdgcn_raw_buffer_store_b128(__builtin_bit_cast(u32x4, pack8bf(h)), rh, (uint32_t)((srow * q.ldh + ub) * 2), 0, 17);
+      if (gout) {
+        const uint32_t pg = park + (uint32_t)(ni * 4 * NT * 16);
+        asm volatile("ds_write_b128 %0, %1" ::"v"(pg), "v"(__builtin_bit_cast(u32x4, pack8bf(gi))) : "memory");
+        asm volatile("ds_write_b128 %0, %1 offset:%2" ::"v"(pg), "v"(__builtin_bit_cast(u32x4, pack8bf(gf))), "n"(NT * 16) : "memory");
+        asm volatile("ds_write_b128 %0, %1 offset:%2" ::"v"(pg), "v"(__builtin_bit_cast(u32x4, pack8bf(gg))), "n"(2 * NT * 16) : "memory");
+        asm volatile("ds_write_b128 %0, %1 offset:%2" ::"v"(pg), "v"(__builtin_bit_cast(u32x4, pack8bf(go))), "n"(3 * NT * 16) : "memory");
+        c_park[ni] = pack8bf(c);
+      }
+      continue;
+    }
+    store8<float>(q.c_out + (long)srow * H + ub, c);
+    store8<T>(hout + (long)srow * q.ldh + ub, h);
+    if (gout) {
+      T* g4 = gout + (long)srow * 4 * H + ub;
+      store8<T>(csave + (long)srow * H + ub, c);
+      if (sgate) { store8<T>(g4, gi); store8<T>(g4 + H, gf); store8<T>(g4 + 2 * H, gg); store8<T>(g4 + 3 * H, go); }
+    }
+  }
+  };
+  if constexpr (PERSIST) {
+    ws_barrier();
+    if (q.add) epilogue(std::true_type{}, std::true_type{}); else epilogue(std::false_type{}, std::true_type{});
+    wait_lgkmcnt<0>();
+    publish();
+    if (gout) {
+#pragma unroll
+      for (int ni = 0; ni < NI; ++ni) {
+        const int row = n0 + wn * (16 * NI) + ni * 16 + lc;
+        const uint32_t pg = park + (uint32_t)(ni * 4 * NT * 16);
+        const u32x4 g0 = lds_read128<0>(pg), g1 = lds_read128<NT * 16>(pg), g2 = lds_read128<2 * NT * 16>(pg), g3 = lds_read128<3 * NT * 16>(pg);
+        wait_lgkmcnt<0>();
+        uint4* g4 = reinterpret_cast<uint4*>(gout + (long)row * 4 * H + ub);
+        *reinterpret_cast<uint4*>(csave + (long)row * H + ub) = c_park[ni];
+        g4[0] = __builtin_bit_cast(uint4, g0); g4[H / 8] = __builtin_bit_cast(uint4, g1);
+        g4[2 * H / 8] = __builtin_bit_cast(uint4, g2); g4[3 * H / 8] = __builtin_bit_cast(uint4, g3);
+      }
+    }
+    return;
+  }
+  const bool full = n0 + BNB <= B;
+  if (q.add) { if (full) epilogue(std::true_type{}, std::true_type{}); else epilogue(std::true_type{}, std::false_type{}); }
+  else { if (full) epilogue(std::false_type{}, std::true_type{}); else epilogue(std::false_type{}, std::false_type{}); }
+}
diff --git a/molecular-vae_amd/csrc/rnn_persist_gm.hip b/molecular-vae_amd/csrc/rnn_persist_gm.hip
--- /dev/null
+++ b/molecular-vae_amd/csrc/rnn_persist_gm.hip
@@ -0,0 +1,189 @@
+#include "common.hpp"
+#include "rnn_gm.hpp"
+#include "persist_common.hpp"
+
+namespace {
+
+constexpr int GL = 4, GH = 1024;
+constexpr int GBN = 256, GNP = GH / 64;
+constexpr int GLDS = 2 * (256 + 256) * KB;
+constexpr int WS_TICKET = 64, WS_DONE = 128;
+
+struct PersistGmArgs {
+  int T, B, NR;
+  uint32_t total;
+  long ldh, add0_tstride;
+  const void* w_ih[GL]; const void* w_hh[GL]; long ldw_ih[GL], ldw_hh[GL];
+  const float* bias[GL];
+  const float* add0;
+  void* hs[GL]; void* cs[GL]; void* gates[GL];
+  float* cstate[GL];
+  uint32_t* status;
+  uint32_t* ticket;
+  uint32_t* done;
+  float* poison;
+  uint32_t spin_limit;
+};
+
+struct Item { int l, t, r, j; };
+
+__device__ __forceinline__ StepTaskF make_task(const PersistGmArgs& a, int l, int t) {
+  const long B = a.B, H = GH;
+  const bf16_t* hl = reinterpret_cast<const bf16_t*>(a.hs[l]);
+  StepTaskF q;
+  q.A0 = l > 0 ? reinterpret_cast<const bf16_t*>(a.hs[l - 1]) + t * B * a.ldh : nullptr;
+  q.lda0 = a.ldh; q.K0 = l > 0 ? GH : 0; q.W0 = a.w_ih[l]; q.ldw0 = a.ldw_ih[l];
+  q.add = l == 0 ? a.add0 + t * a.add0_tstride : nullptr; q.add_ld = 4 * H;
+  q.add_tbl = nullptr; q.add_idx = nullptr; q.add_idx_ld = 0; q.add_rows = 0;
+  q.A1 = t > 0 ? hl + (t - 1) * B * a.ldh : nullptr;
+  q.lda1 = a.ldh; q.K1 = GH; q.W1 = a.w_hh[l]; q.ldw1 = a.ldw_hh[l];
+  q.bias = a.bias[l];
+  q.c_prev = t > 0 ? a.cstate[l] + ((t - 1) & 1) * B * H : nullptr;
+  q.c_out = a.cstate[l] + (t & 1) * B * H;
+  q.c_save = a.cs[l] ? reinterpret_cast<bf16_t*>(a.cs[l]) + t * B * H : nullptr;
+  q.h_out = const_cast<bf16_t*>(hl) + t * B * a.ldh; q.ldh = a.ldh;
+  q.g_out = a.gates[l] ? reinterpret_cast<bf16_t*>(a.gates[l]) + t * B * 4 * H : nullptr;
+  q.hprev_t0 = nullptr; q.t = t; q.h_drop = nullptr; q.dmask = nullptr; q.didx0 = 0;
+  return q;
+}
+
+__device__ __forceinline__ bool wait_inputs(const uint32_t* prev_t, const uint32_t* prev_l, const uint32_t* status, uint32_t limit, int lane) {
+  const uint32_t* f = lane == 0 ? prev_t : lane == 1 ? prev_l : nullptr;
+  for (uint32_t it = 0; it < limit; ++it) {
+    uint32_t v = GNP;
+    if (f) asm volatile("global_load_dword %0, %1, off sc1\n\ts_waitcnt vmcnt(0)" : "=v"(v) : "v"(f) : "memory");
+    if (__builtin_amdgcn_ballot_w64(v < (uint32_t)GNP) == 0ull) return true;
+    if ((it & 63) == 63) {
+      uint32_t s;
+      asm volatile("global_load_dword %0, %1, off sc1\n\ts_waitcnt vmcnt(0)" : "=v"(s) : "v"(status) : "memory");
+      if (__builtin_amdgcn_readfirstlane(s) != 0u) return false;
+    }
+    __builtin_amdgcn_s_sleep(2);
+  }
+  return false;
+}
+
+__global__ __launch_bounds__(512, 1) void lstm_persist_gm_fwd_kernel(PersistGmArgs a) {
+  extern __shared__ __attribute__((aligned(16))) char smem[];
+  __shared__ uint32_t s_tk, s_ok;
+  const int tid = threadIdx.x, lane = tid & 63, wave = __builtin_amdgcn_readfirstlane(tid >> 6);
+  const int T = a.T, NR = a.NR;
+  int d = 0;
+  uint32_t dbase = 0;
+  auto diag_lo = [&](int dd) { return dd - T + 1 > 0 ? dd - T + 1 : 0; };
+  auto diag_n = [&](int dd) { return (uint32_t)(((dd < GL - 1 ? dd : GL - 1) - diag_lo(dd) + 1) * NR * GNP); };
+  auto decode = [&](uint32_t tk) -> Item {
+    while (tk >= dbase + diag_n(d)) { dbase += diag_n(d); ++d; }
+    const int lo = diag_lo(d), nl = (d < GL - 1 ? d : GL - 1) - lo + 1;
+    const int rem = (int)(tk - dbase), j = rem % GNP, rl = rem / GNP, l = lo + rl % nl;
+    return Item{l, d - l, rl / nl, j};
+  };
+  auto counter = [&](int l, int t, int r) { return a.done + ((long)l * T + t) * NR + r; };
+  auto inputs_ready = [&](const Item& it) {
+    return wait_inputs(it.t > 0 ? counter(it.l, it.t - 1, it.r) : nullptr, it.l > 0 ? counter(it.l - 1, it.t, it.r) : nullptr,
+                       a.status, a.spin_limit, lane);
+  };
+
+  if (tid == 0) s_tk = __hip_atomic_fetch_add(a.ticket, 1u, __ATOMIC_RELAXED, __HIP_MEMORY_SCOPE_AGENT);
+  __syncthreads();
+  uint32_t tk = __builtin_amdgcn_readfirstlane(s_tk);
+  Item it = decode(tk < a.total ? tk : 0u);
+  if (wave == 0) {
+    const bool ok = tk >= a.total || inputs_ready(it);
+    if (tid == 0) s_ok = ok ? 1u : 0u;
+  }
+  __syncthreads();
+  bool ok = __builtin_amdgcn_readfirstlane(s_ok) != 0u;
+  while (ok && tk < a.total) {
+    const StepTaskF q = make_task(a, it.l, it.t);
+    const Item done_it = it;
+    auto publish = [&] {
+      uint32_t nxt = 0;
+      if (tid == 0) nxt = __hip_atomic_fetch_add(a.ticket, 1u, __ATOMIC_RELAXED, __HIP_MEMORY_SCOPE_AGENT);
+      wait_vmcnt<0>();
+      if (tid == 0) s_tk = nxt;
+      wait_lgkmcnt<0>();
+      raw_barrier();
+      if (tid == 0) __hip_atomic_fetch_add(counter(done_it.l, done_it.t, done_it.r), 1u, __ATOMIC_RELAXED, __HIP_MEMORY_SCOPE_AGENT);
+      tk = __builtin_amdgcn_readfirstlane(s_tk);
+      if (tk < a.total) it = decode(tk);
+      if (wave == 0) {
+        const bool r = tk >= a.total || inputs_ready(it);
+        if (tid == 0) s_ok = r ? 1u : 0u;
+      }
+    };
+    lstm_fwd_gm_tile<256, 256, 2, false, true>(q, a.B, GH, 0, done_it.r, done_it.j, smem, publish);
+    wait_lgkmcnt<0>();
+    raw_barrier();
+    ok = __builtin_amdgcn_readfirstlane(s_ok) != 0u;
+  }
+  if (!ok && tid == 0) {
+    if (atomicCAS(a.status, 0u, 1u) == 0u) {
+      a.status[1] = blockIdx.x; a.status[2] = (uint32_t)(it.l * 65536 + it.t); a.status[3] = (uint32_t)it.r;
+      if (a.poison) *a.poison = __builtin_nanf("");
+    }
+  }
+}
+
+int persist_gm_knob() {
+  const char* v = mvae_knob("MVAE_PERSIST_GM");
+  return v ? atoi(v) : 1;
+}
+
+}
+
+size_t rnn_persist_gm_fwd_workspace_bytes(const mvae_rnn_fwd_desc* d) { return WS_DONE + (size_t)GL * d->T * (d->B / GBN) * 4; }
+
+bool rnn_persist_gm_fwd_supported(const mvae_rnn_fwd_desc* d) {
+  if (!persist_gm_knob()) return false;
+  if (d->cell != MVAE_CELL_LSTM || d->dtype != MVAE_BF16 || d->layers != GL || d->H != GH || d->T < 1) return false;
+  if (d->B < 1024 || d->B % GBN) return false;
+  if (d->x0 || d->lengths || d->add_table || !d->add0 || (reinterpret_cast<uintptr_t>(d->add0) & 15) || d->add0_tstride % 4) return false;
+  if (d->ldh % 8 || d->ldh < GH) return false;
+  const bool save = d->gates[0] != nullptr;
+  auto al16 = [](const void* p) { return (reinterpret_cast<uintptr_t>(p) & 15) == 0; };
+  for (int l = 0; l < GL; ++l) {
+    if (d->h0[l] || d->hdrop[l] || !d->hs[l] || !d->w_hh[l] || !d->cstate[l] || (l > 0 && !d->w_ih[l])) return false;
+    if ((d->gates[l] != nullptr) != save || (d->cs[l] != nullptr) != save) return false;
+    if (!al16(d->hs[l]) || !al16(d->cstate[l]) || !al16(d->w_hh[l]) || (l > 0 && !al16(d->w_ih[l]))) return false;
+    if ((d->bias[l] && !al16(d->bias[l])) || (save && (!al16(d->gates[l]) || !al16(d->cs[l])))) return false;
+    if (d->ldw_hh[l] % 8 || (l > 0 && d->ldw_ih[l] % 8)) return false;
+    if (4L * GH * d->ldw_hh[l] * 2 >= (1L << 31) || (l > 0 && 4L * GH * d->ldw_ih[l] * 2 >= (1L << 31))) return false;
+  }
+  if ((long)d->B * d->ldh * 2 >= (1L << 31) || (long)d->B * GH * 4 >= (1L << 31)) return false;
+  return true;
+}
+
+int rnn_persist_gm_fwd(const mvae_rnn_fwd_desc* d, void* ws, size_t ws_bytes, hipStream_t st) {
+  if (!rnn_persist_gm_fwd_supported(d)) return MVAE_ERR_UNSUPPORTED;
+  if (!ws || ws_bytes < rnn_persist_gm_fwd_workspace_bytes(d) || (reinterpret_cast<uintptr_t>(ws) & 15)) return MVAE_ERR_WORKSPACE;
+  PersistGmArgs a;
+  a.T = d->T; a.B = d->B; a.NR = d->B / GBN;
+  a.total = (uint32_t)(GL * d->T * a.NR * GNP);
+  a.ldh = d->ldh; a.add0_tstride = d->add0_tstride; a.add0 = d->add0;
+  for (int l = 0; l < GL; ++l) {
+    a.w_ih[l] = d->w_ih[l]; a.w_hh[l] = d->w_hh[l]; a.ldw_ih[l] = d->ldw_ih[l]; a.ldw_hh[l] = d->ldw_hh[l];
+    a.bias[l] = d->bias[l]; a.hs[l] = d->hs[l]; a.cs[l] = d->cs[l]; a.gates[l] = d->gates[l]; a.cstate[l] = d->cstate[l];
+  }
+  char* w = reinterpret_cast<char*>(ws);
+  a.status = reinterpret_cast<uint32_t*>(w);
+  a.ticket = reinterpret_cast<uint32_t*>(w + WS_TICKET);
+  a.done = reinterpret_cast<uint32_t*>(w + WS_DONE);
+  a.poison = d->poison;
+  mvae_tls_status = ws;
+  const char* sp = mvae_knob("MVAE_PERSIST_SPIN");
+  a.spin_limit = sp ? (uint32_t)atoi(sp) : (1u << 17);
+  static std::atomic<int> cus_of[MVAE_MAX_DEVICES];
+  int dev = 0;
+  MVAE_CHECK_HIP(hipGetDevice(&dev));
+  int cus = (dev >= 0 && dev < MVAE_MAX_DEVICES) ? cus_of[dev].load(std::memory_order_acquire) : 0;
+  if (cus == 0) {
+    MVAE_CHECK_HIP(hipFuncSetAttribute(reinterpret_cast<const void*>(lstm_persist_gm_fwd_kernel), hipFuncAttributeMaxDynamicSharedMemorySize, GLDS));
+    MVAE_CHECK_HIP(hipDeviceGetAttribute(&cus, hipDeviceAttributeMultiprocessorCount, dev));
+    if (dev >= 0 && dev < MVAE_MAX_DEVICES) cus_of[dev].store(cus, std::memory_order_release);
+  }
+  MVAE_CHECK_HIP(hipMemsetAsync(ws, 0, rnn_persist_gm_fwd_workspace_bytes(d), st));
+  hipLaunchKernelGGL(lstm_persist_gm_fwd_kernel, dim3(cus), dim3(512), GLDS, st, a);
+  MVAE_CHECK_HIP(hipGetLastError());
+  return MVAE_OK;
+}
diff --git a/molecular-vae_amd/csrc/tile_pipe.hpp b/molecular-vae_amd/csrc/tile_pipe.hpp
--- a/molecular-vae_amd/csrc/tile_pipe.hpp
+++ b/molecular-vae_amd/csrc/tile_pipe.hpp
@@ -138,7 +138,7 @@
   __builtin_amdgcn_sched_barrier(0);
 }
 
-template <int BM, int BN, int NBUF, int NT = 256>
+template <int BM, int BN, int NBUF, int NT = 256, int AUXB = 0>
 __device__ __forceinline__ void pipe_issue_stage(char* smem, const PipeSeg<BM, BN, NT>& s0, const PipeSeg<BM, BN, NT>& s1, int st, int wave) {
 #if defined(__HIP_DEVICE_COMPILE__)
   char* stage = smem + (st % NBUF) * ((BM + BN) * KB);
@@ -154,7 +154,7 @@
 #pragma unroll
   for (int i = 0; i < BN * 8 / NT; ++i) {
     lds_void_t* dst = (lds_void_t*)(stage + BM * KB + (i * NT + wave * 64) * 16);
-    __builtin_amdgcn_raw_ptr_buffer_load_lds(s.rb, dst, 16, s.offB[i] + kbyte, 0, 0, 0);
+    __builtin_amdgcn_raw_ptr_buffer_load_lds(s.rb, dst, 16, s.offB[i] + kbyte, 0, 0, AUXB);
   }
 #endif
 }
@@ -207,10 +207,10 @@
       mma16<T>(__builtin_bit_cast(uint4, a[mi]), __builtin_bit_cast(uint4, b[ni]), acc[mi][ni]);
 }
 
-template <typename T, int BM, int BN, int NBUF, int NT, int MI, int NI, int GA, int M0>
+template <typename T, int BM, int BN, int NBUF, int NT, int MI, int NI, int GA, int M0, int AUXB = 0>
 __device__ __forceinline__ void pipe_block_with_refill(char* smem, const PipeSeg<BM, BN, NT>& s0, const PipeSeg<BM, BN, NT>& s1, bool refill, int st,
                                                        int wave, const u32x4 (&a)[GA], const u32x4 (&b)[NI], f32x4 (&acc)[MI][NI]) {
-  if (refill) pipe_issue_stage<BM, BN, NBUF, NT>(smem, s0, s1, st, wave);
+  if (refill) pipe_issue_stage<BM, BN, NBUF, NT, AUXB>(smem, s0, s1, st, wave);
   SB();
 #pragma unroll
   for (int r = 0; r < GA; ++r)
@@ -225,7 +225,7 @@
     for (int ni = 0; ni < NI; ++ni) mma16<T>(__builtin_bit_cast(uint4, a[r]), __builtin_bit_cast(uint4, b[ni]), acc[M0 + r][ni]);
 }
 
-template <typename T, int BM, int BN, int MI, int NI, int NBUF, int NT>
+template <typename T, int BM, int BN, int MI, int NI, int NBUF, int NT, int AUXB = 0>
 __device__ __forceinline__ void tile_gemm_pipe_all(char* smem, const PipeSeg<BM, BN, NT>& s0, const PipeSeg<BM, BN, NT>& s1, int arow0,
                                                    int brow0, f32x4 (&acc)[MI][NI], int tid) {
   constexpr int STAGE = (BM + BN) * KB;
@@ -251,12 +251,12 @@
   constexpr uint32_t G1 = GA * 16 * KB;
 #pragma unroll
   for (int s = 0; s < NBUF - 1; ++s)
-    if (s < nk) pipe_issue_stage<BM, BN, NBUF, NT>(smem, s0, s1, s, wave);
+    if (s < nk) pipe_issue_stage<BM, BN, NBUF, NT, AUXB>(smem, s0, s1, s, wave);
   u32x4 aX[GA], aY[GA], bh0[NI], bh1[NI];
   if (NBUF - 2 < nk) wait_vmcnt<(NBUF - 2) * LPS>(); else wait_vmcnt<0>();
   ws_barrier();
   int pend = (NBUF - 1 < nk) ? NBUF - 1 : -1;
-  if (pend >= 0 && !late) { pipe_issue_stage<BM, BN, NBUF, NT>(smem, s0, s1, pend, wave); pend = -1; }
+  if (pend >= 0 && !late) { pipe_issue_stage<BM, BN, NBUF, NT, AUXB>(smem, s0, s1, pend, wave); pend = -1; }
   FragRead<0, GA, 16 * KB>::run(aX, lds0 + a_lane[0]);
   FragReadB<0, NI, NI, 0>::run(bh0, lds0 + b_lane[0]);
   for (int kt = 0; kt < nk; ++kt) {
@@ -265,7 +265,7 @@
     FragReadB<0, NI, NI, 0>::run(bh1, st + b_lane[1]);
     wait_lgkmcnt<GA + NI>();
     if constexpr (STAGGER) {
-      pipe_block_with_refill<T, BM, BN, NBUF, NT, MI, NI, GA, 0>(smem, s0, s1, late && pend >= 0, pend, wave, aX, bh0, acc);
+      pipe_block_with_refill<T, BM, BN, NBUF, NT, MI, NI, GA, 0, AUXB>(smem, s0, s1, late && pend >= 0, pend, wave, aX, bh0, acc);
       if (late) pend = -1;
     } else pipe_block<T, MI, NI, GA, 0>(aX, bh0, acc);
     SB();
@@ -285,7 +285,7 @@
       FragRead<0, GA, 16 * KB>::run(aX, sn + a_lane[0]);
       FragReadB<0, NI, NI, 0>::run(bh0, sn + b_lane[0]);
     }
-    pipe_block_with_refill<T, BM, BN, NBUF, NT, MI, NI, GA, GA>(smem, s0, s1, !late && pend >= 0, pend, wave, aY, bh1, acc);
+    pipe_block_with_refill<T, BM, BN, NBUF, NT, MI, NI, GA, GA, AUXB>(smem, s0, s1, !late && pend >= 0, pend, wave, aY, bh1, acc);
     if (!late) pend = -1;
     SB();
   }
```
